# shivangchopra11/MedMoE

Measured on AMD Instinct MI355X. Metric: image-text pairs/sec at global batch 1024, higher is better.
Workload: dtype bf16; 1 GPU; cfg2: ViT-B/16 + 12-layer text tower (frozen), 8 experts top-2, 224x224x3 + 77 tokens, fwd+bwd+clip+Adam; global_batch=1024, per_gpu_batch=1024, parallelism=dp1

## Files before the change

include/medmoe_hip.h:

```cpp
#ifndef MEDMOE_HIP_H
#define MEDMOE_HIP_H
#include <hip/hip_runtime_api.h>
#ifdef __cplusplus
extern "C" {
#endif

int medmoe_attn_fwd(const void* qkv, void* out, float* lse, const unsigned char* key_mask, int B, int N, int H, int head_dim, hipStream_t stream);

int medmoe_attn_bwd(const void* qkv, const void* out, const void* dout, const float* lse, const unsigned char* key_mask, void* dqkv, float* delta, int B, int N, int H, int head_dim, hipStream_t stream);

int medmoe_patchify(const void* img, void* out, int B, int C, int H, int W, int patch, int in_f32, hipStream_t stream);
int medmoe_patchify_ld(const void* img, void* out, int B, int C, int H, int W, int patch, int in_f32, int ld, hipStream_t stream);

int medmoe_init_tokens(void* x, const float* cls, const float* pos, int B, int Nt, int D, hipStream_t stream);

int medmoe_pos_cls_grad(const void* dx, float* dpos, float* dcls, int B, int Nt, int D, hipStream_t stream);

int medmoe_text_embed_ln(const int* ids, const int* type_ids, const float* word, const float* pos, const float* type, const float* gamma, const float* beta, void* out, int B, int T, int D, int vocab, float eps, hipStream_t stream);

int medmoe_text_aggregate(const void* h0, const void* h1, const void* h2, const void* h3, int n_layers, const int* seg, void* word_bf16, float* word_f32, float* sent, int B, int T, int D, hipStream_t stream);

int medmoe_gemm_nt(const void* A, int lda, const void* B, int ldb, void* C, int ldc, int M, int N, int K, const float* bias, const void* residual, int ldr, void* aux, int ldaux, const int* a_rowmap, const int* c_rowmap, const int* tiles, const int* tile_count, int max_tiles, long long strideB, long long strideBias, float alpha, int epi, int out_f32, int col_perm, hipStream_t stream);

int medmoe_gemm_nt_tiles256(const void* A, int lda, const void* B, int ldb, void* C, int ldc, int M, int N, int K, const float* bias, const void* residual, int ldr, void* aux, int ldaux, const int* a_rowmap, const int* c_rowmap, const int* tiles, const int* tile_count, int max_tiles, long long strideB, long long strideBias, float alpha, int epi, int out_f32, int col_perm, hipStream_t stream);

int medmoe_gemm_tn(const void* G, int ldg, const void* X, int ldx, float* dW, int ldw, float* db, int M, int Nn, int Kk, const int* x_rowmap, const int* g_rowmap, const int* row_off, int n_groups, long long strideW, long long strideDb, int nsplit, hipStream_t stream);
int medmoe_gemm_tn_staged(const void* G, int ldg, const void* X, int ldx, float* dW, int ldw, float* db, int M, int Nn, int Kk, float* scratch, long long scratch_floats, hipStream_t stream);

int medmoe_ce_strided(const float* X, float* dX, int rows, int cols, long long rs, long long cs, int label_off, float xscale, float w, int accumulate, float* loss_acc, hipStream_t stream);

int medmoe_soft_xent_strided(const float* X, float* dX, const float* soft, int rows, int cols, long long rs, long long cs, float xscale, float t1, float t2, float w, int accumulate, float* loss_acc, hipStream_t stream);

int medmoe_hardneg_strided(const float* X, float* dX, int rows, int cols, long long rs, long long cs, float margin, float w, int accumulate, float* loss_acc, hipStream_t stream);

int medmoe_rownorm(const float* x, float* n, int rows, int D, hipStream_t stream);

int medmoe_cos_scale(float* S, const float* na, const float* nb, int M, int N, float eps, hipStream_t stream);

int medmoe_cos_scale_bwd(float* dC, const float* C, const float* na, const float* nb, float* ca, float* cb, int M, int N, float eps, hipStream_t stream);

int medmoe_add_rowscaled(float* dst, const float* src, const float* coef, int rows, int D, hipStream_t stream);

int medmoe_words_prep(const void* words, float* wn, void* wT, int Bc, int T, int Tp, int D, hipStream_t stream);

int medmoe_unpad_cast(const float* src, void* dst, int B, int HW, int HWp, int D, hipStream_t stream);

int medmoe_local_pair(const void* ctx, const void* words, const void* gmp, const float* wnorm, const int* cap_lens, const float* gsim, float* sim, void* dS, void* A, void* U, float* att, const void* a1_pre, const float* lse_pre, int B, int Bc, int HW, int T, int D, float temp1, float temp2, float eps, int backward, hipStream_t stream);

int medmoe_local_scores(const void* ctx, const void* words, const int* cap_lens, void* a1, float* lse, int B, int Bc, int HW, int T, int D, hipStream_t stream);

int medmoe_local_pair2(void* a1_io, const float* lse_pre, const void* gmp, const float* wnorm, const int* cap_lens, const float* gsim, float* sim, void* dS, void* U, float* att, int B, int Bc, int HW, int T, float temp1, float temp2, float eps, hipStream_t stream);

int medmoe_scale_blocks(void* X0, void* X1, const float* g, int B, int Bc, int HWp, int Tp, hipStream_t stream);

int medmoe_words_prep_ragged(const void* words, float* wn, void* wT, int Bc, int T, int Tp, int D, const int* col_of_cap, const int* tp_of_cap, long long ldw, hipStream_t stream);
int medmoe_local_scores_ragged(const void* ctx, const void* words, const int* cap_lens, void* a1, float* lse, int B, int Bc, int HW, int T, int D, const int* cap_list, int n_cap, int ntt, long long col_base, long long ldp, hipStream_t stream);
int medmoe_local_pair2_ragged(void* a1_io, const float* lse_pre, const void* gmp, const float* wnorm, const int* cap_lens, const float* gsim, float* sim, void* dS, void* U, int B, int Bc, int HW, int T, float temp1, float temp2, float eps, const int* cap_list, int n_cap, int ntt, long long col_base, long long ldp, hipStream_t stream);
int medmoe_scale_blocks_ragged(void* X0, void* X1, const float* g, int B, int Bc, int HWp, const int* cap_of_chunk, long long ld, hipStream_t stream);

int medmoe_local_pair3(const void* lp, void* dS, void* A, void* U, const float* lse, const void* gm, const float* wnorm, const int* cap_lens, const float* gsim, float* sim, float* att, float* stats, long long stat_rows, int B, int Bc, int HW, int T, float temp1, float temp2, float eps, const int* cap_list, int n_cap, int ntt, long long row_base, long long ld, long long bstride, int pw, float* d2, hipStream_t stream);
int medmoe_local_pair3_wgrad(const void* lp, void* dS, void* A, void* U, const float* lse, const void* gm, const float* wnorm, const int* cap_lens, const float* gsim, float* sim, float* att, float* stats, long long stat_rows, int B, int Bc, int HW, int T, float temp1, float temp2, float eps, const int* cap_list, int n_cap, int ntt, long long row_base, long long ld, long long bstride, int pw, float* d2, float* dwn, hipStream_t stream);
int medmoe_local_scores_t(const void* ctx, const void* words, const int* cap_lens, void* lpT, float* lse, int B, int Bc, int HW, int T, int D, const int* cap_list, int n_cap, int ntt, long long row_base, long long ld, long long bstride, hipStream_t stream);
int medmoe_gemm_tn_cols(const void* G, int ldg, const void* X, int ldx, float* dW, int ldw, int M, int Nn, int Kk, int n_groups, long long gcol_stride, long long xcol_stride, long long strideW, int g_chunk_w, long long g_chunk_stride, hipStream_t stream);

int medmoe_gemm_tn_gram(const void* A, int lda, const float* w, long long w_gstride, int w_ld, float* dW, int ldw, int M, int Nn, int n_groups, long long col_stride, long long strideW, hipStream_t stream);
int medmoe_local_sim_fwd(const void* ctx, const void* words, const int* cap_lens, const void* gm, const float* wnorm, float* sim, int B, int Bc, int HW, int T, int D, float temp1, float temp2, float eps, const int* cap_list, int n_cap, int ntt, hipStream_t stream);
int medmoe_local_sim_chunks(int n);
int medmoe_local_pair3_chunks(int n);
int medmoe_local_pair3_supported(int HW, int T);

int medmoe_segment_map(const void* ids, int ids64, const unsigned char* is_cont, const unsigned char* starts_bracket, int* seg, int* cap, int B, int T, int vocab, int sep_id, hipStream_t stream);

int medmoe_text_aggregate_bwd(const float* d_word, const float* d_sent, const int* seg, void* dH, int B, int T, int D, hipStream_t stream);
int medmoe_text_embed_ln_bwd(const int* ids, const int* type_ids, const float* word, const float* pos, const float* type, const float* gamma, const void* dy, float* dx, float* dgamma, float* dbeta, float* g_word, int B, int T, int D, int vocab, float eps, hipStream_t stream);

int medmoe_text_pack(const unsigned char* mask, int* tok_row, int* src_of_row, int* seq_off, int* count, int B, int T, hipStream_t stream);
int medmoe_text_embed_ln_packed(const int* ids, const int* type_ids, const float* word, const float* pos, const float* type, const float* gamma, const float* beta, void* out, int B, int T, int D, int vocab, float eps, const int* src_of_row, const int* count, hipStream_t stream);
int medmoe_text_aggregate_packed(const void* h0, const void* h1, const void* h2, const void* h3, int n_layers, const int* seg, const int* tok_row, void* word_bf16, float* word_f32, float* sent, int B, int T, int D, hipStream_t stream);
int medmoe_layernorm_fwd_rows(const void* x, const float* gamma, const float* beta, void* y, float* mean, float* rstd, int rows, int D, float eps, int out_f32, const int* rows_dev, hipStream_t stream);
int medmoe_attn_fwd_varlen(const void* qkv, void* out, float* lse, const int* seq_off, int B, int Nmax, int H, int head_dim, hipStream_t stream);
int medmoe_gemm_nt_rows(const void* A, int lda, const void* B, int ldb, void* C, int ldc, int M, int N, int K, const float* bias, const void* residual, int ldr, void* aux, int ldaux, float alpha, int epi, int out_f32, const int* m_dev, hipStream_t stream);

int medmoe_win_attn_fwd(const void* qkv, const float* bias, void* out, float* lse, int B, int H, int W, int C, int heads, int shift, hipStream_t stream);
int medmoe_win_attn_bwd(const void* qkv, const float* bias, const void* dout, const float* lse, void* dqkv, float* dbias, int B, int H, int W, int C, int heads, int shift, hipStream_t stream);
int medmoe_drop_path(const void* branch, const void* res, const float* scale, void* out, int B, long long per_sample, hipStream_t stream);
int medmoe_patch_merge(const void* src, void* dst, int B, int H, int W, int C, int scatter, hipStream_t stream);

int medmoe_preprocess(const void* const* src_ptrs, const int* src_hw, void* dst, int B, int Ho, int Wo, float rescale, const float* mean3, const float* std3, hipStream_t stream);
int medmoe_preprocess_bicubic(const void* const* src_ptrs, const long long* meta, const int* coef, void* tmp, void* dst, void* u8_out, int B, int Ho, int Wo, long long total_src_rows, float rescale, const float* mean3, const float* std3, hipStream_t stream);

int medmoe_local_geometry(int HW, int T, int* HWp, int* Tp, int* GW);
int medmoe_local_fast_path(int HW, int T);

int medmoe_local_gen_fwd_a(const void* lp, const int* cap_lens, void* A, int B, int Bc, int HW, int HWp, int T, int Tp, float temp1, long long ldp, hipStream_t stream);
int medmoe_local_gen_cos(const float* wc, const void* words, const float* wnorm, const int* cap_lens, float* sim, float* stats, float* sume, int B, int Bc, int T, int Tp, int D, float temp2, float eps, long long Kp, hipStream_t stream);
int medmoe_local_gen_dwctx(const float* wc, const void* words, const float* wnorm, const int* cap_lens, const float* gsim, const float* stats, const float* sume, void* dwc, int B, int Bc, int T, int Tp, int D, float temp2, float eps, long long Kp, hipStream_t stream);
int medmoe_local_gen_dwords(const float* wc, const void* words, const float* wnorm, const int* cap_lens, const float* gsim, const float* stats, const float* sume, const float* dws, float* d_words, int B, int Bc, int T, int Tp, int D, float temp2, float eps, long long Kp, hipStream_t stream);
int medmoe_local_gen_bwd_s(const void* lp, const void* A, void* dA_io, const int* cap_lens, int B, int Bc, int HW, int HWp, int T, int Tp, float temp1, long long ldp, hipStream_t stream);
int medmoe_unpad_cast2(const float* src, const float* src2, void* dst, int B, int HW, int HWp, int D, hipStream_t stream);

int medmoe_mean_tokens(const void* x, float* out, int B, int Nt, int D, int t0, int cnt, hipStream_t stream);

int medmoe_broadcast_tokens(const float* g, void* dy, int B, int Nt, int D, int t0, int cnt, float scale, hipStream_t stream);

int medmoe_router_fwd(const float* x, const float* w1, const float* b1, const float* w2, const float* b2, float* h, float* probs, int* idx, float* gates, int B, int Dv, int Hd, int E, int k, hipStream_t stream);

int medmoe_router_bwd(const float* probs, const float* h, const float* w2, const int* idx, const float* dgates, const int* labels, const float* dprobs_ext, float ce_scale, float* dlogits, float* dh, float* loss_acc, int B, int Hd, int E, int k, hipStream_t stream);

int medmoe_router_eval(const float* probs, const int* labels, float* loss_acc, int B, int E, hipStream_t stream);

int medmoe_sgemm(const float* A, const float* Bm, float* C, int M, int N, int K, long long sam, long long sak, long long sbk, long long sbn, long long ldc, float alpha, float beta, hipStream_t stream);

int medmoe_dispatch(const int* idx, int B, int k, int E, int P, int Nt, int* slot_of, int* item_of_slot, int* expert_of_slot, int* row_off, int* tiles, int* tile_count, int max_tiles, int* rowmap, hipStream_t stream);

int medmoe_scale_attn_fwd(const void* G, const void* H1, const float* w2, const float* b2, const int* expert_of_slot, int P, void* out, float* wts, int R, int Do, int Dh, hipStream_t stream);

int medmoe_combine_fwd(const void* expert_out, const int* slot_of, const float* gates, void* img_l, int B, int k, int P, int Do, hipStream_t stream);

int medmoe_scale_attn_bwd(const void* d_img_l, const float* d_img_g, const void* G, const void* H1, const float* wts, const float* w2, const void* expert_out, const int* expert_of_slot, const int* item_of_slot, const float* gates, int k, int P, void* dG, void* dH1, float* dw2, float* db2, float* dgate, int R, int Do, int Dh, hipStream_t stream);

int medmoe_lerp_tokens_fwd(const void* x, void* y, int n, int Pin, int Pout, int D, hipStream_t stream);
int medmoe_lerp_tokens_bwd(const void* dy, const void* relu_aux, void* dx, int n, int Pin, int Pout, int D, hipStream_t stream);
int medmoe_lerp_tokens_bwd2(const void* dy, const void* dy2, const void* relu_aux, void* dx, int n, int Pin, int Pout, int D, hipStream_t stream);

int medmoe_stage_grad_add(const void* dF, const int* slot_of, void* dx, int B, int k, int P, int Nt, int D, hipStream_t stream);

int medmoe_layernorm_fwd(const void* x, const float* gamma, const float* beta, void* y, float* mean, float* rstd, int rows, int D, float eps, int out_f32, hipStream_t stream);

int medmoe_layernorm_bwd(const void* dy, const void* x, const float* mean, const float* rstd, const float* gamma, const void* add, void* dx, float* dgamma, float* dbeta, int rows, int D, hipStream_t stream);

int medmoe_sumsq(const float* g, long long n, float* out, hipStream_t stream);
int medmoe_sumsq_det(const float* g, long long n, float* out, float* scratch, hipStream_t stream);

int medmoe_stream_fork(hipStream_t from, hipStream_t to);

int medmoe_adam_step(float* p, const float* g, float* m, float* v, void* p_bf16, long long n, double lr, double beta1, double beta2, double eps, double weight_decay, int step, const float* grad_normsq, float max_norm, float grad_scale, hipStream_t stream);

int medmoe_adam_groups_step(float* p, const float* g, float* m, float* v, void* p_bf16, long long n, const long long* run_end, const float* run_lr_mult, const float* run_wd_mult, int n_runs, double lr, double beta1, double beta2, double eps, double weight_decay, int decoupled, int step, const float* grad_normsq, float max_norm, float grad_scale, hipStream_t stream);

int medmoe_grad_pack_bf16(const float* g, void* out_bf16, long long n, float scale, hipStream_t stream);
int medmoe_sumsq_det_bf16(const void* g_bf16, long long n, float* out, float* scratch, hipStream_t stream);
int medmoe_adam_step_g16(float* p, const void* g_bf16, float* m, float* v, void* p_bf16, long long n, double lr, double beta1, double beta2, double eps, double weight_decay, int step, const float* grad_normsq, float max_norm, float grad_scale, hipStream_t stream);
int medmoe_adam_groups_step_g16(float* p, const void* g_bf16, float* m, float* v, void* p_bf16, long long n, const long long* run_end, const float* run_lr_mult, const float* run_wd_mult, int n_runs, double lr, double beta1, double beta2, double eps, double weight_decay, int decoupled, int step, const float* grad_normsq, float max_norm, float grad_scale, hipStream_t stream);

int medmoe_adam_step_ema(float* p, const float* g, float* m, float* v, void* p_bf16, long long n, double lr, double beta1, double beta2, double eps, double weight_decay, int step, const float* grad_normsq, float max_norm, float grad_scale, float* ema, float one_minus_decay, hipStream_t stream);
int medmoe_adam_groups_step_ema(float* p, const float* g, float* m, float* v, void* p_bf16, long long n, const long long* run_end, const float* run_lr_mult, const float* run_wd_mult, int n_runs, double lr, double beta1, double beta2, double eps, double weight_decay, int decoupled, int step, const float* grad_normsq, float max_norm, float grad_scale, float* ema, float one_minus_decay, hipStream_t stream);
int medmoe_adam_step_ema_g16(float* p, const void* g_bf16, float* m, float* v, void* p_bf16, long long n, double lr, double beta1, double beta2, double eps, double weight_decay, int step, const float* grad_normsq, float max_norm, float grad_scale, float* ema, float one_minus_decay, hipStream_t stream);
int medmoe_adam_groups_step_ema_g16(float* p, const void* g_bf16, float* m, float* v, void* p_bf16, long long n, const long long* run_end, const float* run_lr_mult, const float* run_wd_mult, int n_runs, double lr, double beta1, double beta2, double eps, double weight_decay, int decoupled, int step, const float* grad_normsq, float max_norm, float grad_scale, float* ema, float one_minus_decay, hipStream_t stream);

int medmoe_cast_bf16(const float* src, void* dst, long long n, hipStream_t stream);

int medmoe_transpose_many(const void* src, void* dst, const long long* table, int n_entries, int max_tiles, hipStream_t stream);

int medmoe_set_option(int key, int value);
int medmoe_last_gemm_nt_kernel(void);

int medmoe_quant_rows_e4m3(const void* x, int ldx, const int* rowmap, const float* colscale, const int* slot_expert, int rows_per_slot, void* q, float* s, int M, int K, hipStream_t stream);
int medmoe_quant_weights_e4m3(const float* w, void* q, void* qT, float* s, int G, int N, int K, hipStream_t stream);
int medmoe_gemm_fp8_grouped(const void* Aq, const float* sa, const void* Bq, const float* sb, const float* bias, void* C, int ldc, const void* residual, const void* aux, const int* tiles, const int* tile_count, int max_tiles, int N, int K, long long strideB, long long strideSb, long long strideBias, int epi, hipStream_t stream);

int medmoe_quant_rows_mx(const void* x, int ldx, const int* rowmap, void* q, void* s, int M, int K, hipStream_t stream);
int medmoe_quant_weights_mx(const float* w, void* q, void* sq, void* qT, void* sT, int G, int N, int K, hipStream_t stream);
int medmoe_gemm_mx_grouped(const void* Aq, const void* sa, const void* Bq, const void* sb, const float* bias, void* C, int ldc, const void* residual, const void* aux, void* Cq, void* Csq, const int* tiles, const int* tile_count, int max_tiles, int N, int K, long long strideB, long long strideSb, long long strideBias, int epi, hipStream_t stream);

int medmoe_dropout_mask(unsigned char* out_u8, long long rows, int cols, int cols_padded, long long seed, long long step, long long site, long long thresh, hipStream_t stream);
int medmoe_dropout_apply(const void* x, void* y, long long rows, int cols, int is_f32, long long seed, long long step, long long site, long long thresh, float scale, hipStream_t stream);
int medmoe_dropout_add_layernorm_fwd(const void* z, const void* residual, const float* gamma, const float* beta, void* x1, void* y, float* mean, float* rstd, int rows, int D, float eps, long long seed, long long step, long long site, long long thresh, float scale, hipStream_t stream);
int medmoe_attn_drop_fwd(const void* qkv, void* out, float* lse, const unsigned char* key_mask, int B, int N, int H, int head_dim, long long seed, long long step, long long site, long long thresh, float scale, hipStream_t stream);
int medmoe_attn_drop_bwd(const void* qkv, const void* out, const void* dout, const float* lse, const unsigned char* key_mask, void* dqkv, float* delta, int B, int N, int H, int head_dim, long long seed, long long step, long long site, long long thresh, float scale, hipStream_t stream);

int medmoe_drop_path_scales(float* out, const double* p_host, int n_sites, int B, long long sample0, long long seed, long long step, long long site0, hipStream_t stream);
int medmoe_scale_add_layernorm_fwd(const void* z, const void* residual, const float* scale, int rows_per_sample, const float* gamma, const float* beta, void* x1, void* y, float* mean, float* rstd, int rows, int D, float eps, hipStream_t stream);

int medmoe_gemm_tn_det(const void* G, int ldg, const void* X, int ldx, float* dW, int ldw, float* db, int M, int Nn, int Kk, const int* x_rowmap, const int* g_rowmap, const int* row_off, int n_groups, long long strideW, long long strideDb, float* scratch, long long scratch_floats, hipStream_t stream);
long long medmoe_gemm_tn_det_scratch(int M, int Nn, int Kk, int x_mapped, int g_mapped, int grouped, int n_groups);
int medmoe_gemm_tn_cols_det(const void* G, int ldg, const void* X, int ldx, float* dW, int ldw, int M, int Nn, int Kk, int n_groups, long long gcol_stride, long long xcol_stride, long long strideW, int g_chunk_w, long long g_chunk_stride, float* scratch, long long scratch_floats, hipStream_t stream);
long long medmoe_gemm_tn_cols_det_scratch(int M, int Nn, int Kk, int n_groups);
int medmoe_gemm_tn_gram_det(const void* A, int lda, const float* w, long long w_gstride, int w_ld, float* dW, int ldw, int M, int Nn, int n_groups, long long col_stride, long long strideW, hipStream_t stream);
int medmoe_layernorm_bwd_det(const void* dy, const void* x, const float* mean, const float* rstd, const float* gamma, const void* add, void* dx, float* dgamma, float* dbeta, int rows, int D, float* scratch, long long scratch_floats, hipStream_t stream);
long long medmoe_layernorm_bwd_det_scratch(int D);
int medmoe_scale_attn_bwd_det(const void* d_img_l, const float* d_img_g, const void* G, const void* H1, const float* wts, const float* w2, const void* expert_out, const int* expert_of_slot, const int* item_of_slot, const float* gates, int k, int P, void* dG, void* dH1, float* dw2, float* db2, float* dgate, int R, int Do, int Dh, const int* row_off, int E, float* scratch, long long scratch_floats, hipStream_t stream);
long long medmoe_scale_attn_bwd_det_scratch(int R, int P, int Dh);
int medmoe_router_bwd_det(const float* probs, const float* h, const float* w2, const int* idx, const float* dgates, const int* labels, const float* dprobs_ext, float ce_scale, float* dlogits, float* dh, float* loss_acc, int B, int Hd, int E, int k, float* parts, hipStream_t stream);
int medmoe_ce_strided_det(const float* X, float* dX, int rows, int cols, long long rs, long long cs, int label_off, float xscale, float w, int accumulate, float* loss_acc, float* parts, hipStream_t stream);
int medmoe_soft_xent_strided_det(const float* X, float* dX, const float* soft, int rows, int cols, long long rs, long long cs, float xscale, float t1, float t2, float w, int accumulate, float* loss_acc, float* parts, hipStream_t stream);
int medmoe_hardneg_strided_det(const float* X, float* dX, int rows, int cols, long long rs, long long cs, float margin, float w, int accumulate, float* loss_acc, float* parts, hipStream_t stream);
int medmoe_cos_scale_bwd_det(float* dC, const float* C, const float* na, const float* nb, float* ca, float* cb, int M, int N, float eps, hipStream_t stream);
long long medmoe_nondet_launches(void);

int medmoe_lora_fwd(const void* X, const void* A, const void* Bw, void* U, void* qkv, int ldq, int M, int D, int n, int c0, int c1, int c2, float s, long long seed, long long step, long long site, long long thresh, float scale, hipStream_t stream);
int medmoe_lora_bwd_dx(const void* dqkv, int ldq, const void* Bt, const void* At, void* dU, void* dy, int M, int D, int n, int c0, int c1, int c2, float s, long long seed, long long step, long long site, long long thresh, float scale, hipStream_t stream);
int medmoe_lora_bwd_wgrad(const void* dqkv, int ldq, const void* X, const void* U, const void* dU, float* gA, float* gB, float* scratch, long long scratch_floats, int M, int D, int n, int c0, int c1, int c2, float s, long long seed, long long step, long long site, long long thresh, float scale, hipStream_t stream);
long long medmoe_lora_wgrad_scratch(int M, int D, int n);
int medmoe_lora_merge(void* W, int ldw, const void* A, const void* Bw, int D, int n, int c0, int c1, int c2, float s, hipStream_t stream);

int medmoe_attn_bwd_varlen(const void* qkv, const void* out, const void* dout, const float* lse, const int* seq_off, void* dqkv, float* delta, int B, int Nmax, int H, int head_dim, hipStream_t stream);
int medmoe_layernorm_bwd_rows(const void* dy, const void* x, const float* mean, const float* rstd, const float* gamma, const void* add, void* dx, float* dgamma, float* dbeta, int rows, int D, const int* rows_dev, hipStream_t stream);
int medmoe_text_aggregate_bwd_packed(const float* d_word, const float* d_sent, const int* seg, const int* src_of_row, const int* count, void* dH, int B, int T, int D, hipStream_t stream);
int medmoe_text_embed_ln_bwd_packed(const int* ids, const int* type_ids, const float* word, const float* pos, const float* type, const float* gamma, const void* dy, float* dx, float* dgamma, float* dbeta, float* g_word, int B, int T, int D, int vocab, float eps, const int* src_of_row, const int* count, hipStream_t stream);
int medmoe_lora_fwd_rows(const void* X, const void* A, const void* Bw, void* U, void* qkv, int ldq, int M, int D, int n, int c0, int c1, int c2, float s, long long seed, long long step, long long site, long long thresh, float scale, const int* rows_dev, hipStream_t stream);
int medmoe_lora_bwd_dx_rows(const void* dqkv, int ldq, const void* Bt, const void* At, void* dU, void* dy, int M, int D, int n, int c0, int c1, int c2, float s, long long seed, long long step, long long site, long long thresh, float scale, const int* rows_dev, hipStream_t stream);
int medmoe_lora_bwd_wgrad_rows(const void* dqkv, int ldq, const void* X, const void* U, const void* dU, float* gA, float* gB, float* scratch, long long scratch_floats, int M, int D, int n, int c0, int c1, int c2, float s, long long seed, long long step, long long site, long long thresh, float scale, const int* rows_dev, hipStream_t stream);

#ifdef __cplusplus
}
#endif
#endif
```

medmoe_amd/csrc/attention.hip:

```cpp
#include "common.h"

#define HD 64

__device__ __forceinline__ int tpos(int r) {
  const int o = r & 31;
  return (r & ~31) + (((o & 15) >> 2) << 3) + ((o >> 4) << 2) + (o & 3);
}

template <int CNT, int RT>
__device__ __forceinline__ void fill_rowmajor(char* lds, const bf16_t* src, long long row_stride, int n_valid, int tid) {
  constexpr int PER = (CNT + RT - 1) / RT;
  uint4 v[PER];
#pragma unroll
  for (int i = 0; i < PER; ++i) {
    const int idx = min(tid + i * RT, CNT - 1);
    const int row = idx >> 3, c = idx & 7;
    v[i] = *(const uint4*)(src + (long long)min(row, n_valid - 1) * row_stride + c * 8);
  }
#pragma unroll
  for (int i = 0; i < PER; ++i) {
    const int idx = tid + i * RT;
    const int row = idx >> 3, c = idx & 7;
    if (idx < CNT) *(uint4*)(lds + row * 128 + ((c ^ (row & 7)) << 4)) = v[i];
  }
}

__device__ __forceinline__ void fill_transposed(char* lds, const bf16_t* src, long long row_stride, int n_valid,
                                                int stride_bytes, int tid) {
  for (int i = tid; i < (64 * stride_bytes) / 16; i += 256) *(uint4*)(lds + i * 16) = make_uint4(0, 0, 0, 0);
  __syncthreads();
  for (int idx = tid; idx < n_valid * 8; idx += 256) {
    const int row = idx >> 3, c = idx & 7;
    const uint4 v = *(const uint4*)(src + (long long)row * row_stride + c * 8);
    const uint32_t w[4] = {v.x, v.y, v.z, v.w};
    const int pos = tpos(row);
#pragma unroll
    for (int e = 0; e < 4; ++e) {
      *(bf16_t*)(lds + (c * 8 + 2 * e) * stride_bytes + pos * 2) = (bf16_t)(w[e] & 0xffff);
      *(bf16_t*)(lds + (c * 8 + 2 * e + 1) * stride_bytes + pos * 2) = (bf16_t)(w[e] >> 16);
    }
  }
}

__device__ __forceinline__ bf16x8_t tr_frag(const char* img, int row0, int col0, int lane) {
  const int q = (lane & 15) >> 2, pp = lane & 3;
  const int ra = row0 + 4 * (lane >> 4) + q, rb = ra + 16;
  const int col = col0 + 4 * pp;
  const int ch = col >> 3, within = (col & 7) << 1;
  const bf16x4_t lo = __builtin_amdgcn_ds_read_tr16_b64_v4bf16(
      (__attribute__((address_space(3))) bf16x4_t*)(img + ra * 128 + ((ch ^ (ra & 7)) << 4) + within));
  const bf16x4_t hi = __builtin_amdgcn_ds_read_tr16_b64_v4bf16(
      (__attribute__((address_space(3))) bf16x4_t*)(img + rb * 128 + ((ch ^ (rb & 7)) << 4) + within));
  return __builtin_shufflevector(lo, hi, 0, 1, 2, 3, 4, 5, 6, 7);
}

__device__ __forceinline__ bf16x8_t load_frag_global(const bf16_t* base, long long row_stride, int row, int chunk) {
  const uint4 v = *(const uint4*)(base + (long long)row * row_stride + chunk * 8);
  return __builtin_bit_cast(bf16x8_t, v);
}

__device__ __forceinline__ bf16x8_t pack_frag(const f32x4_t& a, const f32x4_t& b) {
  uint4 v;
  v.x = pack2bf(a[0], a[1]); v.y = pack2bf(a[2], a[3]);
  v.z = pack2bf(b[0], b[1]); v.w = pack2bf(b[2], b[3]);
  return __builtin_bit_cast(bf16x8_t, v);
}

template <int NKT>
struct AttnGeom {
  static constexpr int NKP = NKT * 16;
  static constexpr int KS = (NKT + 1) / 2;
  static constexpr int RMROWS = KS * 32;
  static constexpr int RM_BYTES = RMROWS * 128;
  static constexpr int FILL = RMROWS * 8;
};

#ifdef ATTN_TIMING
__device__ unsigned long long g_attn_timing[8];
#define ATTN_T(...) __VA_ARGS__
#else
#define ATTN_T(...)
#endif

template <int NKT, bool MASKED, int RT>
__global__ __launch_bounds__(RT, RT == 256 ? 2 : 4) void attn_fwd_kernel(const bf16_t* __restrict__ qkv, bf16_t* __restrict__ out,
                                                         float* __restrict__ lse, const unsigned char* __restrict__ key_mask,
                                                         int Nmax, int H, float scale, const int* __restrict__ seq_off) {
  using G = AttnGeom<NKT>;
  constexpr int CH = 8;
  constexpr int NCH = (NKT + CH - 1) / CH;
  __shared__ __attribute__((aligned(16))) char smem[2 * G::RM_BYTES + G::NKP * 4];
  char* sK = smem;
  char* sV = smem + G::RM_BYTES;
  float* sMask = (float*)(smem + 2 * G::RM_BYTES);
  const int tid = threadIdx.x, lane = tid & 63, wid = tid >> 6;
  const int b = blockIdx.x / H, h = blockIdx.x - b * H;
  const int D = H * HD;
  const long long rs = 3LL * D;
  const long long row0 = seq_off ? (long long)seq_off[b] : (long long)b * Nmax;
  const int N = seq_off ? max(1, min(seq_off[b + 1] - seq_off[b], Nmax)) : Nmax;
  const bf16_t* base = qkv + row0 * rs + h * HD;

  fill_rowmajor<G::FILL, RT>(sK, base + D, rs, N, tid);
  fill_rowmajor<G::FILL, RT>(sV, base + 2 * D, rs, N, tid);
  for (int k = tid; k < G::NKP; k += RT)
    sMask[k] = (k < N && (!key_mask || key_mask[(long long)b * Nmax + k])) ? 0.f : -INFINITY;
  __syncthreads();

  const int fr = lane & 15, g = lane >> 4;
  const int nqb = (N + 15) >> 4;
  const float c2 = scale * 1.44269504088896f;
  bf16x8_t qf[2], qn[2];
  {
    const int qc0 = min(wid * 16 + fr, N - 1);
    qf[0] = load_frag_global(base, rs, qc0, g);
    qf[1] = load_frag_global(base, rs, qc0, 4 + g);
  }
  for (int qb = wid; qb < nqb; qb += RT / 64) {
    const int q = qb * 16 + fr;
    {
      const int qcn = min((qb + RT / 64) * 16 + fr, N - 1);
      qn[0] = load_frag_global(base, rs, qcn, g);
      qn[1] = load_frag_global(base, rs, qcn, 4 + g);
    }
    float m = -INFINITY, lp = 0.f;
    f32x4_t o[4];
#pragma unroll
    for (int nd = 0; nd < 4; ++nd) o[nd] = (f32x4_t){0.f, 0.f, 0.f, 0.f};
#pragma unroll 1
    for (int c = 0; c < NCH; ++c) {
      const int kt0 = c * CH;
      f32x4_t s[CH];
#pragma unroll
      for (int u = 0; u < CH; ++u) {
        s[u] = (f32x4_t){0.f, 0.f, 0.f, 0.f};
        if (kt0 + u < NKT) {
          const char* kr = sK + ((kt0 + u) * 16 + fr) * 128;
#pragma unroll
          for (int ks = 0; ks < 2; ++ks) {
            const bf16x8_t kf = *(const bf16x8_t*)(kr + (((ks * 4 + g) ^ (fr & 7)) << 4));
            s[u] = __builtin_amdgcn_mfma_f32_16x16x32_bf16(kf, qf[ks], s[u], 0, 0, 0);
          }
        }
      }
      float alpha;
      f32x2_t l2 = {0.f, 0.f};
      if constexpr (MASKED) {
        float bm = -INFINITY;
#pragma unroll
        for (int u = 0; u < CH; ++u)
          if (kt0 + u < NKT) {
            const float4 mk = *(const float4*)(sMask + (kt0 + u) * 16 + g * 4);
            const f32x2_t t0 = (f32x2_t){s[u][0], s[u][1]} * c2 + (f32x2_t){mk.x, mk.y};
            const f32x2_t t1 = (f32x2_t){s[u][2], s[u][3]} * c2 + (f32x2_t){mk.z, mk.w};
            s[u][0] = t0[0]; s[u][1] = t0[1]; s[u][2] = t1[0]; s[u][3] = t1[1];
            bm = fmaxf(fmaxf(bm, fmaxf(t0[0], t0[1])), fmaxf(t1[0], t1[1]));
          }
        bm = fmaxf(bm, __shfl_xor(bm, 16, 64));
        bm = fmaxf(bm, __shfl_xor(bm, 32, 64));
        const float mn = fmaxf(m, bm);
        const float ms = (mn == -INFINITY) ? 0.f : mn;
        alpha = __builtin_amdgcn_exp2f(m - ms);
        m = mn;
#pragma unroll
        for (int u = 0; u < CH; ++u)
          if (kt0 + u < NKT) {
            const f32x2_t d0 = (f32x2_t){s[u][0], s[u][1]} - ms, d1 = (f32x2_t){s[u][2], s[u][3]} - ms;
            const f32x2_t e0 = {__builtin_amdgcn_exp2f(d0[0]), __builtin_amdgcn_exp2f(d0[1])};
            const f32x2_t e1 = {__builtin_amdgcn_exp2f(d1[0]), __builtin_amdgcn_exp2f(d1[1])};
            s[u][0] = e0[0]; s[u][1] = e0[1]; s[u][2] = e1[0]; s[u][3] = e1[1];
            l2 += e0 + e1;
          }
      } else {
        float bm = fmaxf(fmaxf(s[0][0], s[0][1]), fmaxf(s[0][2], s[0][3]));
#pragma unroll
        for (int u = 1; u < CH; ++u)
          if (kt0 + u < NKT) bm = fmaxf(fmaxf(bm, fmaxf(s[u][0], s[u][1])), fmaxf(s[u][2], s[u][3]));
        bm = fmaxf(bm, __shfl_xor(bm, 16, 64));
        bm = fmaxf(bm, __shfl_xor(bm, 32, 64));
        const float mn = fmaxf(m, bm * c2);
        alpha = __builtin_amdgcn_exp2f(m - mn);
        m = mn;
        const float nm = -mn;
#pragma unroll
        for (int u = 0; u < CH; ++u)
          if (kt0 + u < NKT) {
            const f32x2_t d0 = (f32x2_t){s[u][0], s[u][1]} * c2 + nm, d1 = (f32x2_t){s[u][2], s[u][3]} * c2 + nm;
            f32x2_t e0 = {__builtin_amdgcn_exp2f(d0[0]), __builtin_amdgcn_exp2f(d0[1])};
            f32x2_t e1 = {__builtin_amdgcn_exp2f(d1[0]), __builtin_amdgcn_exp2f(d1[1])};
            if ((kt0 + u) * 16 + 16 > N) {
              const int k0 = (kt0 + u) * 16 + g * 4;
              e0[0] = k0 < N ? e0[0] : 0.f; e0[1] = k0 + 1 < N ? e0[1] : 0.f;
              e1[0] = k0 + 2 < N ? e1[0] : 0.f; e1[1] = k0 + 3 < N ? e1[1] : 0.f;
            }
            s[u][0] = e0[0]; s[u][1] = e0[1]; s[u][2] = e1[0]; s[u][3] = e1[1];
            l2 += e0 + e1;
          }
      }
      lp = lp * alpha + l2[0] + l2[1];
#pragma unroll
      for (int nd = 0; nd < 4; ++nd) {
        if (c > 0) o[nd] *= alpha;
#pragma unroll
        for (int t = 0; t < CH / 2; ++t)
          if (kt0 + 2 * t < NKT) {
            const bf16x8_t pf = pack_frag(s[2 * t], s[2 * t + 1]);
            const bf16x8_t vf = tr_frag(sV, (kt0 + 2 * t) * 16, nd * 16, lane);
            o[nd] = __builtin_amdgcn_mfma_f32_16x16x32_bf16(vf, pf, o[nd], 0, 0, 0);
          }
      }
    }
    float l = lp;
    l += __shfl_xor(l, 16, 64);
    l += __shfl_xor(l, 32, 64);
    const float inv = l > 0.f ? 1.f / l : 0.f;
    if (q < N) {
      if (g == 0) lse[((long long)b * H + h) * Nmax + q] = (m + __log2f(l)) * 0.693147180559945f;
#pragma unroll
      for (int nd = 0; nd < 4; ++nd) {
        const f32x4_t v = o[nd] * inv;
        uint2 pk; pk.x = pack2bf(v[0], v[1]); pk.y = pack2bf(v[2], v[3]);
        *(uint2*)(out + (row0 + q) * D + h * HD + nd * 16 + g * 4) = pk;
      }
    }
    qf[0] = qn[0]; qf[1] = qn[1];
  }
}

template <int NKT, bool MASKED, int RT>
__global__ __launch_bounds__(RT, 4) void attn_bwd_dq_kernel(const bf16_t* __restrict__ qkv, const bf16_t* __restrict__ o,
                                                          const bf16_t* __restrict__ dout, const float* __restrict__ lse,
                                                          const unsigned char* __restrict__ key_mask,
                                                          bf16_t* __restrict__ dqkv, float* __restrict__ delta,
                                                          int Nmax, int H, float scale, const int* __restrict__ seq_off) {
  using G = AttnGeom<NKT>;
  __shared__ __attribute__((aligned(16))) char smem[2 * G::RM_BYTES + G::NKP * 4];
  char* sK = smem;
  char* sV = smem + G::RM_BYTES;
  float* sMask = (float*)(smem + 2 * G::RM_BYTES);
  const int tid = threadIdx.x, lane = tid & 63, wid = tid >> 6;
  const int b = blockIdx.x / H, h = blockIdx.x - b * H;
  const int D = H * HD;
  const long long rs = 3LL * D;
  const long long row0 = seq_off ? (long long)seq_off[b] : (long long)b * Nmax;
  const int N = seq_off ? max(1, min(seq_off[b + 1] - seq_off[b], Nmax)) : Nmax;
  const bf16_t* base = qkv + row0 * rs + h * HD;
  const bf16_t* obase = o + row0 * D + h * HD;
  const bf16_t* dobase = dout + row0 * D + h * HD;

  fill_rowmajor<G::FILL, RT>(sK, base + D, rs, N, tid);
  fill_rowmajor<G::FILL, RT>(sV, base + 2 * D, rs, N, tid);
  for (int k = tid; k < G::NKP; k += RT)
    sMask[k] = (k < N && (!key_mask || key_mask[(long long)b * Nmax + k])) ? 0.f : -INFINITY;
  __syncthreads();

  const int fr = lane & 15, g = lane >> 4;
  const int nqb = (N + 15) >> 4;
  bf16x8_t qf[2], dof[2], of[2], qn[2], don[2], on[2];
  {
    const int qc0 = min(wid * 16 + fr, N - 1);
#pragma unroll
    for (int ks = 0; ks < 2; ++ks) {
      qf[ks] = load_frag_global(base, rs, qc0, ks * 4 + g);
      dof[ks] = load_frag_global(dobase, D, qc0, ks * 4 + g);
      of[ks] = load_frag_global(obase, D, qc0, ks * 4 + g);
    }
  }
  for (int qb = wid; qb < nqb; qb += RT / 64) {
    const int q = qb * 16 + fr;
    const int qc = min(q, N - 1);
    {
      const int qcn = min((qb + RT / 64) * 16 + fr, N - 1);
#pragma unroll
      for (int ks = 0; ks < 2; ++ks) {
        qn[ks] = load_frag_global(base, rs, qcn, ks * 4 + g);
        don[ks] = load_frag_global(dobase, D, qcn, ks * 4 + g);
        on[ks] = load_frag_global(obase, D, qcn, ks * 4 + g);
      }
    }
    float dl = 0.f;
#pragma unroll
    for (int ks = 0; ks < 2; ++ks)
#pragma unroll
      for (int e = 0; e < 8; ++e) dl += (float)dof[ks][e] * (float)of[ks][e];
    dl += __shfl_xor(dl, 16, 64);
    dl += __shfl_xor(dl, 32, 64);
    const float c2 = scale * 1.44269504088896f;
    const float nL2 = -lse[((long long)b * H + h) * Nmax + qc] * 1.44269504088896f;
    if (g == 0 && q < N) delta[((long long)b * H + h) * Nmax + q] = dl;

    f32x4_t acc[4];
#pragma unroll
    for (int nd = 0; nd < 4; ++nd) acc[nd] = (f32x4_t){0.f, 0.f, 0.f, 0.f};
#pragma unroll 1
    for (int t = 0; t < G::KS; ++t) {
      f32x4_t ds[2];
#pragma unroll
      for (int u = 0; u < 2; ++u) {
        const int kt = 2 * t + u;
        ds[u] = (f32x4_t){0.f, 0.f, 0.f, 0.f};
        if (kt < NKT) {
          f32x4_t s = {0.f, 0.f, 0.f, 0.f}, dp = {0.f, 0.f, 0.f, 0.f};
          const char* kr = sK + (kt * 16 + fr) * 128;
          const char* vr = sV + (kt * 16 + fr) * 128;
#pragma unroll
          for (int ks = 0; ks < 2; ++ks) {
            const int off = ((ks * 4 + g) ^ (fr & 7)) << 4;
            s = __builtin_amdgcn_mfma_f32_16x16x32_bf16(*(const bf16x8_t*)(kr + off), qf[ks], s, 0, 0, 0);
            dp = __builtin_amdgcn_mfma_f32_16x16x32_bf16(*(const bf16x8_t*)(vr + off), dof[ks], dp, 0, 0, 0);
          }
          if (MASKED || kt * 16 + 16 > N) {
            const float4 mk = *(const float4*)(sMask + kt * 16 + g * 4);
            const float mkv[4] = {mk.x, mk.y, mk.z, mk.w};
#pragma unroll
            for (int r = 0; r < 4; ++r) ds[u][r] = __builtin_amdgcn_exp2f(s[r] * c2 + (mkv[r] + nL2)) * (dp[r] - dl);
          } else {
            const f32x2_t t0 = (f32x2_t){s[0], s[1]} * c2 + nL2, t1 = (f32x2_t){s[2], s[3]} * c2 + nL2;
            const f32x2_t g0 = (f32x2_t){dp[0], dp[1]} - dl, g1 = (f32x2_t){dp[2], dp[3]} - dl;
            const f32x2_t d0 = (f32x2_t){__builtin_amdgcn_exp2f(t0[0]), __builtin_amdgcn_exp2f(t0[1])} * g0;
            const f32x2_t d1 = (f32x2_t){__builtin_amdgcn_exp2f(t1[0]), __builtin_amdgcn_exp2f(t1[1])} * g1;
            ds[u] = (f32x4_t){d0[0], d0[1], d1[0], d1[1]};
          }
        }
      }
      const bf16x8_t dsf = pack_frag(ds[0], ds[1]);
#pragma unroll
      for (int nd = 0; nd < 4; ++nd) {
        const bf16x8_t ktf = tr_frag(sK, t * 32, nd * 16, lane);
        acc[nd] = __builtin_amdgcn_mfma_f32_16x16x32_bf16(ktf, dsf, acc[nd], 0, 0, 0);
      }
    }
    if (q < N) {
#pragma unroll
      for (int nd = 0; nd < 4; ++nd) {
        const f32x4_t v = acc[nd] * scale;
        uint2 pk; pk.x = pack2bf(v[0], v[1]); pk.y = pack2bf(v[2], v[3]);
        *(uint2*)(dqkv + (row0 + q) * rs + h * HD + nd * 16 + g * 4) = pk;
      }
    }
#pragma unroll
    for (int ks = 0; ks < 2; ++ks) { qf[ks] = qn[ks]; dof[ks] = don[ks]; of[ks] = on[ks]; }
  }
}

template <int NKT, int RT>
__global__ __launch_bounds__(RT, 4) void attn_bwd_dkv_kernel(const bf16_t* __restrict__ qkv, const bf16_t* __restrict__ dout,
                                                           const float* __restrict__ lse, const float* __restrict__ delta,
                                                           const unsigned char* __restrict__ key_mask,
                                                           bf16_t* __restrict__ dqkv, int Nmax, int H, float scale,
                                                           const int* __restrict__ seq_off) {
  using G = AttnGeom<NKT>;
  __shared__ __attribute__((aligned(16))) char smem[2 * G::RM_BYTES + G::NKP * 12];
  char* sQ = smem;
  char* sDO = smem + G::RM_BYTES;
  float* sMask = (float*)(smem + 2 * G::RM_BYTES);
  float* sLse = sMask + G::NKP;
  float* sDelta = sLse + G::NKP;
  const int tid = threadIdx.x, lane = tid & 63, wid = tid >> 6;
  const int b = blockIdx.x / H, h = blockIdx.x - b * H;
  const int D = H * HD;
  const long long rs = 3LL * D;
  const long long row0 = seq_off ? (long long)seq_off[b] : (long long)b * Nmax;
  const int N = seq_off ? max(1, min(seq_off[b + 1] - seq_off[b], Nmax)) : Nmax;
  const bf16_t* base = qkv + row0 * rs + h * HD;
  const bf16_t* dobase = dout + row0 * D + h * HD;

  fill_rowmajor<G::FILL, RT>(sQ, base, rs, N, tid);
  fill_rowmajor<G::FILL, RT>(sDO, dobase, D, N, tid);
  for (int k = tid; k < G::NKP; k += RT) {
    const bool valid = k < N;
    sMask[k] = (valid && (!key_mask || key_mask[(long long)b * Nmax + k])) ? 0.f : -INFINITY;
    sLse[k] = valid ? lse[((long long)b * H + h) * Nmax + k] * 1.44269504088896f : INFINITY;
    sDelta[k] = valid ? delta[((long long)b * H + h) * Nmax + k] : 0.f;
  }
  __syncthreads();

  const int fr = lane & 15, g = lane >> 4;
  const int nkb = (N + 15) >> 4;
  bf16x8_t kf[2], vf[2], kn[2], vn[2];
  {
    const int kc0 = min(wid * 16 + fr, N - 1);
#pragma unroll
    for (int ks = 0; ks < 2; ++ks) {
      kf[ks] = load_frag_global(base + D, rs, kc0, ks * 4 + g);
      vf[ks] = load_frag_global(base + 2 * D, rs, kc0, ks * 4 + g);
    }
  }
  for (int kb = wid; kb < nkb; kb += RT / 64) {
    const int key = kb * 16 + fr;
    {
      const int kcn = min((kb + RT / 64) * 16 + fr, N - 1);
#pragma unroll
      for (int ks = 0; ks < 2; ++ks) {
        kn[ks] = load_frag_global(base + D, rs, kcn, ks * 4 + g);
        vn[ks] = load_frag_global(base + 2 * D, rs, kcn, ks * 4 + g);
      }
    }
    const float mk = sMask[kb * 16 + fr];
    const float c2 = scale * 1.44269504088896f;
    f32x4_t dk[4], dv[4];
#pragma unroll
    for (int nd = 0; nd < 4; ++nd) { dk[nd] = (f32x4_t){0.f, 0.f, 0.f, 0.f}; dv[nd] = (f32x4_t){0.f, 0.f, 0.f, 0.f}; }

#pragma unroll 1
    for (int t = 0; t < G::KS; ++t) {
      f32x4_t pp[2], dss[2];
#pragma unroll
      for (int u = 0; u < 2; ++u) {
        const int qt = 2 * t + u;
        if (qt < NKT) {
          f32x4_t s = {0.f, 0.f, 0.f, 0.f}, dp = {0.f, 0.f, 0.f, 0.f};
          const char* qr = sQ + (qt * 16 + fr) * 128;
          const char* dr = sDO + (qt * 16 + fr) * 128;
#pragma unroll
          for (int ks = 0; ks < 2; ++ks) {
            const int off = ((ks * 4 + g) ^ (fr & 7)) << 4;
            s = __builtin_amdgcn_mfma_f32_16x16x32_bf16(*(const bf16x8_t*)(qr + off), kf[ks], s, 0, 0, 0);
            dp = __builtin_amdgcn_mfma_f32_16x16x32_bf16(*(const bf16x8_t*)(dr + off), vf[ks], dp, 0, 0, 0);
          }
          const float4 L4 = *(const float4*)(sLse + qt * 16 + g * 4);
          const float4 D4 = *(const float4*)(sDelta + qt * 16 + g * 4);
          const float Lv[4] = {L4.x, L4.y, L4.z, L4.w}, Dv[4] = {D4.x, D4.y, D4.z, D4.w};
          const f32x2_t t0 = (f32x2_t){s[0], s[1]} * c2 + (mk - (f32x2_t){Lv[0], Lv[1]});
          const f32x2_t t1 = (f32x2_t){s[2], s[3]} * c2 + (mk - (f32x2_t){Lv[2], Lv[3]});
          const f32x2_t p0 = {__builtin_amdgcn_exp2f(t0[0]), __builtin_amdgcn_exp2f(t0[1])};
          const f32x2_t p1 = {__builtin_amdgcn_exp2f(t1[0]), __builtin_amdgcn_exp2f(t1[1])};
          const f32x2_t d0 = p0 * ((f32x2_t){dp[0], dp[1]} - (f32x2_t){Dv[0], Dv[1]});
          const f32x2_t d1 = p1 * ((f32x2_t){dp[2], dp[3]} - (f32x2_t){Dv[2], Dv[3]});
          pp[u] = (f32x4_t){p0[0], p0[1], p1[0], p1[1]};
          dss[u] = (f32x4_t){d0[0], d0[1], d1[0], d1[1]};
        } else {
          pp[u] = (f32x4_t){0.f, 0.f, 0.f, 0.f};
          dss[u] = (f32x4_t){0.f, 0.f, 0.f, 0.f};
        }
      }
      const bf16x8_t pf = pack_frag(pp[0], pp[1]);
      const bf16x8_t dsf = pack_frag(dss[0], dss[1]);
#pragma unroll
      for (int nd = 0; nd < 4; ++nd) {
        const bf16x8_t dot = tr_frag(sDO, t * 32, nd * 16, lane);
        const bf16x8_t qt_ = tr_frag(sQ, t * 32, nd * 16, lane);
        dv[nd] = __builtin_amdgcn_mfma_f32_16x16x32_bf16(dot, pf, dv[nd], 0, 0, 0);
        dk[nd] = __builtin_amdgcn_mfma_f32_16x16x32_bf16(qt_, dsf, dk[nd], 0, 0, 0);
      }
    }
    if (key < N) {
      bf16_t* row = dqkv + (row0 + key) * rs + h * HD;
#pragma unroll
      for (int nd = 0; nd < 4; ++nd) {
        const f32x4_t kv = dk[nd] * scale;
        uint2 pk; pk.x = pack2bf(kv[0], kv[1]); pk.y = pack2bf(kv[2], kv[3]);
        *(uint2*)(row + D + nd * 16 + g * 4) = pk;
        pk.x = pack2bf(dv[nd][0], dv[nd][1]); pk.y = pack2bf(dv[nd][2], dv[nd][3]);
        *(uint2*)(row + 2 * D + nd * 16 + g * 4) = pk;
      }
    }
#pragma unroll
    for (int ks = 0; ks < 2; ++ks) { kf[ks] = kn[ks]; vf[ks] = vn[ks]; }
  }
}

#define SB 64
#define SB_BYTES (SB * 128)

__device__ __forceinline__ void stage_load(uint4 (&v)[2], const bf16_t* src, long long row_stride, int row0, int n_valid, int tid) {
#pragma unroll
  for (int i = 0; i < 2; ++i) {
    const int idx = tid + i * 256;
    const int row = idx >> 3, c = idx & 7;
    v[i] = *(const uint4*)(src + (long long)min(row0 + row, n_valid - 1) * row_stride + c * 8);
  }
}
__device__ __forceinline__ void stage_store(char* lds, const uint4 (&v)[2], int tid) {
#pragma unroll
  for (int i = 0; i < 2; ++i) {
    const int idx = tid + i * 256;
    const int row = idx >> 3, c = idx & 7;
    *(uint4*)(lds + row * 128 + ((c ^ (row & 7)) << 4)) = v[i];
  }
}
__device__ __forceinline__ bf16x8_t rm_frag(const char* img, int t16, int ks, int fr, int g) {
  return *(const bf16x8_t*)(img + (t16 * 16 + fr) * 128 + (((ks * 4 + g) ^ (fr & 7)) << 4));
}

template <bool MASKED>
__global__ __launch_bounds__(256) void attn_fwd_stream_kernel(const bf16_t* __restrict__ qkv, bf16_t* __restrict__ out,
                                                              float* __restrict__ lse, const unsigned char* __restrict__ key_mask,
                                                              int N, int H, int QB, float scale) {
  __shared__ __attribute__((aligned(16))) char smem[4 * SB_BYTES + 2 * SB * 4];
  const int tid = threadIdx.x, lane = tid & 63, wid = tid >> 6;
  const int fr = lane & 15, g = lane >> 4;
  const int id = xcd_remap(blockIdx.x, gridDim.x);
  const int bh = id / QB, qc = id - bh * QB;
  const int b = bh / H, h = bh - b * H;
  const int D = H * HD;
  const long long rs = 3LL * D;
  const bf16_t* base = qkv + (long long)b * N * rs + h * HD;
  const int q0 = qc * 64 + wid * 16;
  const bool active = q0 < N;
  const int q = q0 + fr;
  bf16x8_t qf[2];
  {
    const int qr = min(q, N - 1);
    qf[0] = load_frag_global(base, rs, qr, g);
    qf[1] = load_frag_global(base, rs, qr, 4 + g);
  }
  const int nkb = (N + SB - 1) / SB;
  auto bufK = [&](int i) { return smem + i * 2 * SB_BYTES; };
  auto bufV = [&](int i) { return smem + i * 2 * SB_BYTES + SB_BYTES; };
  float* sMaskAll = (float*)(smem + 4 * SB_BYTES);
  auto mask_of = [&](int key) -> float { return (key < N && (!key_mask || key_mask[(long long)b * N + key])) ? 0.f : -INFINITY; };
  uint4 kr[2], vr[2];
  stage_load(kr, base + D, rs, 0, N, tid);
  stage_load(vr, base + 2 * D, rs, 0, N, tid);
  stage_store(bufK(0), kr, tid); stage_store(bufV(0), vr, tid);
  if (tid < SB) sMaskAll[tid] = mask_of(tid);
  __syncthreads();

  const float c2 = scale * 1.44269504088896f;
  float m = -INFINITY, lp = 0.f;
  f32x4_t o[4];
#pragma unroll
  for (int nd = 0; nd < 4; ++nd) o[nd] = (f32x4_t){0.f, 0.f, 0.f, 0.f};
  for (int kb = 0; kb < nkb; ++kb) {
    const int cur = kb & 1;
    const bool more = kb + 1 < nkb;
    float mnext = 0.f;
    if (more) {
      stage_load(kr, base + D, rs, (kb + 1) * SB, N, tid);
      stage_load(vr, base + 2 * D, rs, (kb + 1) * SB, N, tid);
      if (tid < SB) mnext = mask_of((kb + 1) * SB + tid);
    }
    if (active) {
      const char* sK = bufK(cur);
      const char* sV = bufV(cur);
      const float* sM = sMaskAll + cur * SB;
      f32x4_t s[4];
#pragma unroll
      for (int kt = 0; kt < 4; ++kt) {
        s[kt] = (f32x4_t){0.f, 0.f, 0.f, 0.f};
#pragma unroll
        for (int ks = 0; ks < 2; ++ks) s[kt] = __builtin_amdgcn_mfma_f32_16x16x32_bf16(rm_frag(sK, kt, ks, fr, g), qf[ks], s[kt], 0, 0, 0);
      }
      float alpha;
      f32x2_t l2 = {0.f, 0.f};
      if constexpr (MASKED) {
        float bm = -INFINITY;
#pragma unroll
        for (int kt = 0; kt < 4; ++kt) {
          const float4 mk = *(const float4*)(sM + kt * 16 + g * 4);
          const f32x2_t t0 = (f32x2_t){s[kt][0], s[kt][1]} * c2 + (f32x2_t){mk.x, mk.y};
          const f32x2_t t1 = (f32x2_t){s[kt][2], s[kt][3]} * c2 + (f32x2_t){mk.z, mk.w};
          s[kt][0] = t0[0]; s[kt][1] = t0[1]; s[kt][2] = t1[0]; s[kt][3] = t1[1];
          bm = fmaxf(fmaxf(bm, fmaxf(t0[0], t0[1])), fmaxf(t1[0], t1[1]));
        }
        bm = fmaxf(bm, __shfl_xor(bm, 16, 64));
        bm = fmaxf(bm, __shfl_xor(bm, 32, 64));
        const float mn = fmaxf(m, bm);
        const float ms = (mn == -INFINITY) ? 0.f : mn;
        alpha = __builtin_amdgcn_exp2f(m - ms);
        m = mn;
#pragma unroll
        for (int kt = 0; kt < 4; ++kt) {
          const f32x2_t d0 = (f32x2_t){s[kt][0], s[kt][1]} - ms, d1 = (f32x2_t){s[kt][2], s[kt][3]} - ms;
          const f32x2_t e0 = {__builtin_amdgcn_exp2f(d0[0]), __builtin_amdgcn_exp2f(d0[1])};
          const f32x2_t e1 = {__builtin_amdgcn_exp2f(d1[0]), __builtin_amdgcn_exp2f(d1[1])};
          s[kt][0] = e0[0]; s[kt][1] = e0[1]; s[kt][2] = e1[0]; s[kt][3] = e1[1];
          l2 += e0 + e1;
        }
      } else {
        float bm = fmaxf(fmaxf(s[0][0], s[0][1]), fmaxf(s[0][2], s[0][3]));
#pragma unroll
        for (int kt = 1; kt < 4; ++kt) bm = fmaxf(fmaxf(bm, fmaxf(s[kt][0], s[kt][1])), fmaxf(s[kt][2], s[kt][3]));
        bm = fmaxf(bm, __shfl_xor(bm, 16, 64));
        bm = fmaxf(bm, __shfl_xor(bm, 32, 64));
        const float mn = fmaxf(m, bm * c2);
        alpha = __builtin_amdgcn_exp2f(m - mn);
        m = mn;
        const float nm = -mn;
        const bool tail = kb * SB + SB > N;
#pragma unroll
        for (int kt = 0; kt < 4; ++kt) {
          const f32x2_t d0 = (f32x2_t){s[kt][0], s[kt][1]} * c2 + nm, d1 = (f32x2_t){s[kt][2], s[kt][3]} * c2 + nm;
          f32x2_t e0 = {__builtin_amdgcn_exp2f(d0[0]), __builtin_amdgcn_exp2f(d0[1])};
          f32x2_t e1 = {__builtin_amdgcn_exp2f(d1[0]), __builtin_amdgcn_exp2f(d1[1])};
          if (tail) {
            const int k0 = kb * SB + kt * 16 + g * 4;
            e0[0] = k0 < N ? e0[0] : 0.f; e0[1] = k0 + 1 < N ? e0[1] : 0.f;
            e1[0] = k0 + 2 < N ? e1[0] : 0.f; e1[1] = k0 + 3 < N ? e1[1] : 0.f;
          }
          s[kt][0] = e0[0]; s[kt][1] = e0[1]; s[kt][2] = e1[0]; s[kt][3] = e1[1];
          l2 += e0 + e1;
        }
      }
      lp = lp * alpha + l2[0] + l2[1];
      bf16x8_t pf[2];
      pf[0] = pack_frag(s[0], s[1]);
      pf[1] = pack_frag(s[2], s[3]);
#pragma unroll
      for (int nd = 0; nd < 4; ++nd) {
        o[nd] *= alpha;
#pragma unroll
        for (int t = 0; t < 2; ++t) o[nd] = __builtin_amdgcn_mfma_f32_16x16x32_bf16(tr_frag(sV, t * 32, nd * 16, lane), pf[t], o[nd], 0, 0, 0);
      }
    }
    if (more) {
      stage_store(bufK(cur ^ 1), kr, tid); stage_store(bufV(cur ^ 1), vr, tid);
      if (tid < SB) sMaskAll[(cur ^ 1) * SB + tid] = mnext;
    }
    __syncthreads();
  }
  if (!active) return;
  float l = lp;
  l += __shfl_xor(l, 16, 64);
  l += __shfl_xor(l, 32, 64);
  const float inv = l > 0.f ? 1.f / l : 0.f;
  if (q < N) {
    if (g == 0) lse[((long long)b * H + h) * N + q] = (m + __log2f(l)) * 0.693147180559945f;
#pragma unroll
    for (int nd = 0; nd < 4; ++nd) {
      const f32x4_t v = o[nd] * inv;
      uint2 pk; pk.x = pack2bf(v[0], v[1]); pk.y = pack2bf(v[2], v[3]);
      *(uint2*)(out + ((long long)b * N + q) * D + h * HD + nd * 16 + g * 4) = pk;
    }
  }
}

template <bool MASKED>
__global__ __launch_bounds__(256) void attn_bwd_dq_stream_kernel(const bf16_t* __restrict__ qkv, const bf16_t* __restrict__ o,
                                                                 const bf16_t* __restrict__ dout, const float* __restrict__ lse,
                                                                 const unsigned char* __restrict__ key_mask,
                                                                 bf16_t* __restrict__ dqkv, float* __restrict__ delta,
                                                                 int N, int H, int QB, float scale) {
  __shared__ __attribute__((aligned(16))) char smem[4 * SB_BYTES + 2 * SB * 4];
  const int tid = threadIdx.x, lane = tid & 63, wid = tid >> 6;
  const int fr = lane & 15, g = lane >> 4;
  const int id = xcd_remap(blockIdx.x, gridDim.x);
  const int bh = id / QB, qc = id - bh * QB;
  const int b = bh / H, h = bh - b * H;
  const int D = H * HD;
  const long long rs = 3LL * D;
  const bf16_t* base = qkv + (long long)b * N * rs + h * HD;
  const bf16_t* obase = o + (long long)b * N * D + h * HD;
  const bf16_t* dobase = dout + (long long)b * N * D + h * HD;
  const int q0 = qc * 64 + wid * 16;
  const bool active = q0 < N;
  const int q = q0 + fr, qr = min(q, N - 1);
  bf16x8_t qf[2], dof[2];
  float dl = 0.f;
  {
    bf16x8_t of[2];
#pragma unroll
    for (int ks = 0; ks < 2; ++ks) {
      qf[ks] = load_frag_global(base, rs, qr, ks * 4 + g);
      dof[ks] = load_frag_global(dobase, D, qr, ks * 4 + g);
      of[ks] = load_frag_global(obase, D, qr, ks * 4 + g);
    }
#pragma unroll
    for (int ks = 0; ks < 2; ++ks)
#pragma unroll
      for (int e = 0; e < 8; ++e) dl += (float)dof[ks][e] * (float)of[ks][e];
    dl += __shfl_xor(dl, 16, 64);
    dl += __shfl_xor(dl, 32, 64);
  }
  const float c2 = scale * 1.44269504088896f;
  const float nL2 = -lse[((long long)b * H + h) * N + qr] * 1.44269504088896f;
  if (active && g == 0 && q < N) delta[((long long)b * H + h) * N + q] = dl;

  const int nkb = (N + SB - 1) / SB;
  auto bufK = [&](int i) { return smem + i * 2 * SB_BYTES; };
  auto bufV = [&](int i) { return smem + i * 2 * SB_BYTES + SB_BYTES; };
  float* sMaskAll = (float*)(smem + 4 * SB_BYTES);
  auto mask_of = [&](int key) -> float { return (key < N && (!key_mask || key_mask[(long long)b * N + key])) ? 0.f : -INFINITY; };
  uint4 kr[2], vr[2];
  stage_load(kr, base + D, rs, 0, N, tid);
  stage_load(vr, base + 2 * D, rs, 0, N, tid);
  stage_store(bufK(0), kr, tid); stage_store(bufV(0), vr, tid);
  if (tid < SB) sMaskAll[tid] = mask_of(tid);
  __syncthreads();
  f32x4_t acc[4];
#pragma unroll
  for (int nd = 0; nd < 4; ++nd) acc[nd] = (f32x4_t){0.f, 0.f, 0.f, 0.f};
  for (int kb = 0; kb < nkb; ++kb) {
    const int cur = kb & 1;
    const bool more = kb + 1 < nkb;
    float mnext = 0.f;
    if (more) {
      stage_load(kr, base + D, rs, (kb + 1) * SB, N, tid);
      stage_load(vr, base + 2 * D, rs, (kb + 1) * SB, N, tid);
      if (tid < SB) mnext = mask_of((kb + 1) * SB + tid);
    }
    if (active) {
      const char* sK = bufK(cur);
      const char* sV = bufV(cur);
      const float* sM = sMaskAll + cur * SB;
      f32x4_t ds[4];
#pragma unroll
      for (int kt = 0; kt < 4; ++kt) {
        f32x4_t s = {0.f, 0.f, 0.f, 0.f}, dp = {0.f, 0.f, 0.f, 0.f};
#pragma unroll
        for (int ks = 0; ks < 2; ++ks) {
          s = __builtin_amdgcn_mfma_f32_16x16x32_bf16(rm_frag(sK, kt, ks, fr, g), qf[ks], s, 0, 0, 0);
          dp = __builtin_amdgcn_mfma_f32_16x16x32_bf16(rm_frag(sV, kt, ks, fr, g), dof[ks], dp, 0, 0, 0);
        }
        if (MASKED || kb * SB + SB > N) {
          const float4 mk = *(const float4*)(sM + kt * 16 + g * 4);
          const float mkv[4] = {mk.x, mk.y, mk.z, mk.w};
#pragma unroll
          for (int r = 0; r < 4; ++r) ds[kt][r] = __builtin_amdgcn_exp2f(s[r] * c2 + (mkv[r] + nL2)) * (dp[r] - dl);
        } else {
          const f32x2_t t0 = (f32x2_t){s[0], s[1]} * c2 + nL2, t1 = (f32x2_t){s[2], s[3]} * c2 + nL2;
          const f32x2_t d0 = (f32x2_t){__builtin_amdgcn_exp2f(t0[0]), __builtin_amdgcn_exp2f(t0[1])} * ((f32x2_t){dp[0], dp[1]} - dl);
          const f32x2_t d1 = (f32x2_t){__builtin_amdgcn_exp2f(t1[0]), __builtin_amdgcn_exp2f(t1[1])} * ((f32x2_t){dp[2], dp[3]} - dl);
          ds[kt] = (f32x4_t){d0[0], d0[1], d1[0], d1[1]};
        }
      }
      const bf16x8_t dsf0 = pack_frag(ds[0], ds[1]), dsf1 = pack_frag(ds[2], ds[3]);
#pragma unroll
      for (int nd = 0; nd < 4; ++nd) {
        acc[nd] = __builtin_amdgcn_mfma_f32_16x16x32_bf16(tr_frag(sK, 0, nd * 16, lane), dsf0, acc[nd], 0, 0, 0);
        acc[nd] = __builtin_amdgcn_mfma_f32_16x16x32_bf16(tr_frag(sK, 32, nd * 16, lane), dsf1, acc[nd], 0, 0, 0);
      }
    }
    if (more) {
      stage_store(bufK(cur ^ 1), kr, tid); stage_store(bufV(cur ^ 1), vr, tid);
      if (tid < SB) sMaskAll[(cur ^ 1) * SB + tid] = mnext;
    }
    __syncthreads();
  }
  if (active && q < N) {
#pragma unroll
    for (int nd = 0; nd < 4; ++nd) {
      const f32x4_t v = acc[nd] * scale;
      uint2 pk; pk.x = pack2bf(v[0], v[1]); pk.y = pack2bf(v[2], v[3]);
      *(uint2*)(dqkv + ((long long)b * N + q) * rs + h * HD + nd * 16 + g * 4) = pk;
    }
  }
}

__global__ __launch_bounds__(256) void attn_bwd_dkv_stream_kernel(const bf16_t* __restrict__ qkv, const bf16_t* __restrict__ dout,
                                                                  const float* __restrict__ lse, const float* __restrict__ delta,
                                                                  const unsigned char* __restrict__ key_mask,
                                                                  bf16_t* __restrict__ dqkv, int N, int H, int QB, float scale) {
  __shared__ __attribute__((aligned(16))) char smem[4 * SB_BYTES + 4 * SB * 4];
  const int tid = threadIdx.x, lane = tid & 63, wid = tid >> 6;
  const int fr = lane & 15, g = lane >> 4;
  const int id = xcd_remap(blockIdx.x, gridDim.x);
  const int bh = id / QB, kc = id - bh * QB;
  const int b = bh / H, h = bh - b * H;
  const int D = H * HD;
  const long long rs = 3LL * D;
  const bf16_t* base = qkv + (long long)b * N * rs + h * HD;
  const bf16_t* dobase = dout + (long long)b * N * D + h * HD;
  const float* lrow = lse + ((long long)b * H + h) * N;
  const float* drow = delta + ((long long)b * H + h) * N;
  const int k0 = kc * 64 + wid * 16;
  const bool active = k0 < N;
  const int key = k0 + fr, kr_ = min(key, N - 1);
  bf16x8_t kf[2], vf[2];
#pragma unroll
  for (int ks = 0; ks < 2; ++ks) {
    kf[ks] = load_frag_global(base + D, rs, kr_, ks * 4 + g);
    vf[ks] = load_frag_global(base + 2 * D, rs, kr_, ks * 4 + g);
  }
  const float mk = (key < N && (!key_mask || key_mask[(long long)b * N + key])) ? 0.f : -INFINITY;
  const float c2 = scale * 1.44269504088896f;
  const int nqb = (N + SB - 1) / SB;
  auto bufQ = [&](int i) { return smem + i * 2 * SB_BYTES; };
  auto bufD = [&](int i) { return smem + i * 2 * SB_BYTES + SB_BYTES; };
  float* sL = (float*)(smem + 4 * SB_BYTES);
  float* sDl = sL + 2 * SB;
  uint4 qr[2], dr[2];
  stage_load(qr, base, rs, 0, N, tid);
  stage_load(dr, dobase, D, 0, N, tid);
  stage_store(bufQ(0), qr, tid); stage_store(bufD(0), dr, tid);
  if (tid < SB) { sL[tid] = tid < N ? lrow[tid] * 1.44269504088896f : INFINITY; sDl[tid] = tid < N ? drow[tid] : 0.f; }
  __syncthreads();
  f32x4_t dk[4], dv[4];
#pragma unroll
  for (int nd = 0; nd < 4; ++nd) { dk[nd] = (f32x4_t){0.f, 0.f, 0.f, 0.f}; dv[nd] = (f32x4_t){0.f, 0.f, 0.f, 0.f}; }
  for (int qb = 0; qb < nqb; ++qb) {
    const int cur = qb & 1;
    const bool more = qb + 1 < nqb;
    float ln = 0.f, dn = 0.f;
    if (more) {
      stage_load(qr, base, rs, (qb + 1) * SB, N, tid);
      stage_load(dr, dobase, D, (qb + 1) * SB, N, tid);
      if (tid < SB) {
        const int qq = (qb + 1) * SB + tid;
        ln = qq < N ? lrow[qq] * 1.44269504088896f : INFINITY; dn = qq < N ? drow[qq] : 0.f;
      }
    }
    if (active) {
      const char* sQ = bufQ(cur);
      const char* sDO = bufD(cur);
      const float* cL = sL + cur * SB;
      const float* cD = sDl + cur * SB;
      f32x4_t pp[4], dss[4];
#pragma unroll
      for (int qt = 0; qt < 4; ++qt) {
        f32x4_t s = {0.f, 0.f, 0.f, 0.f}, dp = {0.f, 0.f, 0.f, 0.f};
#pragma unroll
        for (int ks = 0; ks < 2; ++ks) {
          s = __builtin_amdgcn_mfma_f32_16x16x32_bf16(rm_frag(sQ, qt, ks, fr, g), kf[ks], s, 0, 0, 0);
          dp = __builtin_amdgcn_mfma_f32_16x16x32_bf16(rm_frag(sDO, qt, ks, fr, g), vf[ks], dp, 0, 0, 0);
        }
        const float4 L4 = *(const float4*)(cL + qt * 16 + g * 4);
        const float4 D4 = *(const float4*)(cD + qt * 16 + g * 4);
        const float Lv[4] = {L4.x, L4.y, L4.z, L4.w}, Dv[4] = {D4.x, D4.y, D4.z, D4.w};
        const f32x2_t t0 = (f32x2_t){s[0], s[1]} * c2 + (mk - (f32x2_t){Lv[0], Lv[1]});
        const f32x2_t t1 = (f32x2_t){s[2], s[3]} * c2 + (mk - (f32x2_t){Lv[2], Lv[3]});
        const f32x2_t p0 = {__builtin_amdgcn_exp2f(t0[0]), __builtin_amdgcn_exp2f(t0[1])};
        const f32x2_t p1 = {__builtin_amdgcn_exp2f(t1[0]), __builtin_amdgcn_exp2f(t1[1])};
        const f32x2_t d0 = p0 * ((f32x2_t){dp[0], dp[1]} - (f32x2_t){Dv[0], Dv[1]});
        const f32x2_t d1 = p1 * ((f32x2_t){dp[2], dp[3]} - (f32x2_t){Dv[2], Dv[3]});
        pp[qt] = (f32x4_t){p0[0], p0[1], p1[0], p1[1]};
        dss[qt] = (f32x4_t){d0[0], d0[1], d1[0], d1[1]};
      }
#pragma unroll
      for (int t = 0; t < 2; ++t) {
        const bf16x8_t pf = pack_frag(pp[2 * t], pp[2 * t + 1]);
        const bf16x8_t dsf = pack_frag(dss[2 * t], dss[2 * t + 1]);
#pragma unroll
        for (int nd = 0; nd < 4; ++nd) {
          dv[nd] = __builtin_amdgcn_mfma_f32_16x16x32_bf16(tr_frag(sDO, t * 32, nd * 16, lane), pf, dv[nd], 0, 0, 0);
          dk[nd] = __builtin_amdgcn_mfma_f32_16x16x32_bf16(tr_frag(sQ, t * 32, nd * 16, lane), dsf, dk[nd], 0, 0, 0);
        }
      }
    }
    if (more) {
      stage_store(bufQ(cur ^ 1), qr, tid); stage_store(bufD(cur ^ 1), dr, tid);
      if (tid < SB) { sL[(cur ^ 1) * SB + tid] = ln; sDl[(cur ^ 1) * SB + tid] = dn; }
    }
    __syncthreads();
  }
  if (active && key < N) {
    bf16_t* row = dqkv + ((long long)b * N + key) * rs + h * HD;
#pragma unroll
    for (int nd = 0; nd < 4; ++nd) {
      const f32x4_t kv = dk[nd] * scale;
      uint2 pk; pk.x = pack2bf(kv[0], kv[1]); pk.y = pack2bf(kv[2], kv[3]);
      *(uint2*)(row + D + nd * 16 + g * 4) = pk;
      pk.x = pack2bf(dv[nd][0], dv[nd][1]); pk.y = pack2bf(dv[nd][2], dv[nd][3]);
      *(uint2*)(row + 2 * D + nd * 16 + g * 4) = pk;
    }
  }
}

int g_attn_resident = 1;
int g_attn_rt13 = 0;

static int pick_nkt(int N) {
  if (N <= 80) return 5;
  if (N <= 208) return 13;
  if (N <= 272) return 17;
  if (N <= 592) return 37;
  return 0;
}

template <int K, int RT>
static void launch_fwd(const void* qkv, void* out, float* lse, const unsigned char* key_mask, int B, int N, int H, float scale, hipStream_t stream) {
  if (key_mask) hipLaunchKernelGGL((attn_fwd_kernel<K, true, RT>), dim3(B * H), dim3(RT), 0, stream, (const bf16_t*)qkv, (bf16_t*)out, lse, key_mask, N, H, scale, (const int*)nullptr);
  else hipLaunchKernelGGL((attn_fwd_kernel<K, false, RT>), dim3(B * H), dim3(RT), 0, stream, (const bf16_t*)qkv, (bf16_t*)out, lse, key_mask, N, H, scale, (const int*)nullptr);
}
template <int K, int RT>
static void launch_bwd(const void* qkv, const void* out, const void* dout, const float* lse, const unsigned char* key_mask, void* dqkv,
                       float* delta, int B, int N, int H, float scale, hipStream_t stream) {
  if (key_mask) hipLaunchKernelGGL((attn_bwd_dq_kernel<K, true, RT>), dim3(B * H), dim3(RT), 0, stream, (const bf16_t*)qkv, (const bf16_t*)out,
                                   (const bf16_t*)dout, lse, key_mask, (bf16_t*)dqkv, delta, N, H, scale, (const int*)nullptr);
  else hipLaunchKernelGGL((attn_bwd_dq_kernel<K, false, RT>), dim3(B * H), dim3(RT), 0, stream, (const bf16_t*)qkv, (const bf16_t*)out,
                          (const bf16_t*)dout, lse, key_mask, (bf16_t*)dqkv, delta, N, H, scale, (const int*)nullptr);
  hipLaunchKernelGGL((attn_bwd_dkv_kernel<K, RT>), dim3(B * H), dim3(RT), 0, stream, (const bf16_t*)qkv, (const bf16_t*)dout, lse, delta,
                     key_mask, (bf16_t*)dqkv, N, H, scale, (const int*)nullptr);
}

extern "C" int medmoe_attn_fwd(const void* qkv, void* out, float* lse, const unsigned char* key_mask,
                               int B, int N, int H, int head_dim, hipStream_t stream) {
  if (!qkv || !out || !lse) return MM_ERR_ARG;
  if (head_dim != HD || B <= 0 || H <= 0 || N <= 0) return MM_ERR_SHAPE;
  const int nkt = pick_nkt(N);
  const float scale = 0.125f;
  if (!g_attn_resident || !nkt) {
    const int QB = (N + SB - 1) / SB;
    if (key_mask) hipLaunchKernelGGL(attn_fwd_stream_kernel<true>, dim3(B * H * QB), dim3(256), 0, stream, (const bf16_t*)qkv, (bf16_t*)out,
                                     lse, key_mask, N, H, QB, scale);
    else hipLaunchKernelGGL(attn_fwd_stream_kernel<false>, dim3(B * H * QB), dim3(256), 0, stream, (const bf16_t*)qkv, (bf16_t*)out,
                            lse, key_mask, N, H, QB, scale);
    return mm_check_launch();
  }
  if (nkt == 5) launch_fwd<5, 256>(qkv, out, lse, key_mask, B, N, H, scale, stream);
  else if (nkt == 13 && (g_attn_rt13 == 448 || (g_attn_rt13 == 0 && B * H >= 4096))) launch_fwd<13, 448>(qkv, out, lse, key_mask, B, N, H, scale, stream);
  else if (nkt == 13) launch_fwd<13, 512>(qkv, out, lse, key_mask, B, N, H, scale, stream);
  else if (nkt == 17) launch_fwd<17, 512>(qkv, out, lse, key_mask, B, N, H, scale, stream);
  else launch_fwd<37, 1024>(qkv, out, lse, key_mask, B, N, H, scale, stream);
  return mm_check_launch();
}

extern "C" int medmoe_attn_fwd_varlen(const void* qkv, void* out, float* lse, const int* seq_off, int B, int Nmax, int H, int head_dim,
                                      hipStream_t stream) {
  if (!qkv || !out || !lse || !seq_off) return MM_ERR_ARG;
  if (head_dim != HD || B <= 0 || H <= 0 || Nmax <= 0 || Nmax > 80) return MM_ERR_SHAPE;
  hipLaunchKernelGGL((attn_fwd_kernel<5, false, 256>), dim3(B * H), dim3(256), 0, stream, (const bf16_t*)qkv, (bf16_t*)out, lse,
                     (const unsigned char*)nullptr, Nmax, H, 0.125f, seq_off);
  return mm_check_launch();
}

extern "C" int medmoe_attn_bwd(const void* qkv, const void* out, const void* dout, const float* lse,
                               const unsigned char* key_mask, void* dqkv, float* delta, int B, int N,
                               int H, int head_dim, hipStream_t stream) {
  if (!qkv || !out || !dout || !lse || !dqkv || !delta) return MM_ERR_ARG;
  if (head_dim != HD || B <= 0 || H <= 0 || N <= 0) return MM_ERR_SHAPE;
  const int nkt = pick_nkt(N);
  const float scale = 0.125f;
  if (!g_attn_resident || !nkt) {
    const int QB = (N + SB - 1) / SB;
    if (key_mask) hipLaunchKernelGGL(attn_bwd_dq_stream_kernel<true>, dim3(B * H * QB), dim3(256), 0, stream, (const bf16_t*)qkv,
                                     (const bf16_t*)out, (const bf16_t*)dout, lse, key_mask, (bf16_t*)dqkv, delta, N, H, QB, scale);
    else hipLaunchKernelGGL(attn_bwd_dq_stream_kernel<false>, dim3(B * H * QB), dim3(256), 0, stream, (const bf16_t*)qkv,
                            (const bf16_t*)out, (const bf16_t*)dout, lse, key_mask, (bf16_t*)dqkv, delta, N, H, QB, scale);
    hipLaunchKernelGGL(attn_bwd_dkv_stream_kernel, dim3(B * H * QB), dim3(256), 0, stream, (const bf16_t*)qkv, (const bf16_t*)dout,
                       lse, delta, key_mask, (bf16_t*)dqkv, N, H, QB, scale);
    return mm_check_launch();
  }
  if (nkt == 5) launch_bwd<5, 256>(qkv, out, dout, lse, key_mask, dqkv, delta, B, N, H, scale, stream);
  else if (nkt == 13 && g_attn_rt13 == 448) launch_bwd<13, 448>(qkv, out, dout, lse, key_mask, dqkv, delta, B, N, H, scale, stream);
  else if (nkt == 13) launch_bwd<13, 512>(qkv, out, dout, lse, key_mask, dqkv, delta, B, N, H, scale, stream);
  else if (nkt == 17) launch_bwd<17, 512>(qkv, out, dout, lse, key_mask, dqkv, delta, B, N, H, scale, stream);
  else launch_bwd<37, 1024>(qkv, out, dout, lse, key_mask, dqkv, delta, B, N, H, scale, stream);
  return mm_check_launch();
}

extern "C" int medmoe_attn_bwd_varlen(const void* qkv, const void* out, const void* dout, const float* lse, const int* seq_off, void* dqkv,
                                      float* delta, int B, int Nmax, int H, int head_dim, hipStream_t stream) {
  if (!qkv || !out || !dout || !lse || !seq_off || !dqkv || !delta) return MM_ERR_ARG;
  if (head_dim != HD || B <= 0 || H <= 0 || Nmax <= 0 || Nmax > 80) return MM_ERR_SHAPE;
  hipLaunchKernelGGL((attn_bwd_dq_kernel<5, false, 256>), dim3(B * H), dim3(256), 0, stream, (const bf16_t*)qkv, (const bf16_t*)out,
                     (const bf16_t*)dout, lse, (const unsigned char*)nullptr, (bf16_t*)dqkv, delta, Nmax, H, 0.125f, seq_off);
  hipLaunchKernelGGL((attn_bwd_dkv_kernel<5, 256>), dim3(B * H), dim3(256), 0, stream, (const bf16_t*)qkv, (const bf16_t*)dout, lse, delta,
                     (const unsigned char*)nullptr, (bf16_t*)dqkv, Nmax, H, 0.125f, seq_off);
  return mm_check_launch();
}
```

medmoe_amd/csrc/gemm.hip:

```cpp
#include "common.h"
#include "det_plan.h"
#include <utility>

#define BM 128
#define BN 128
#define BK 64

__device__ __attribute__((aligned(256))) bf16_t g_zero_page[2048];

struct GemmNTArgs {
  const bf16_t* A; const bf16_t* B; void* C;
  const float* bias; const bf16_t* residual; bf16_t* aux;
  const int* a_rowmap; const int* c_rowmap; const int4* tiles; const int* tile_count;
  long long strideB; long long strideBias;
  int M, N, K, lda, ldb, ldc, ldr, ldaux;
  int n_tiles_n, max_tiles_m;
  float alpha; int epi; int out_f32; int col_perm;
  const int* m_dev;
};

static int g_use_nt256 = 1, g_use_nt512 = 1, g_use_tn512 = 1, g_tn_rows = 1024, g_nt_max_grid = 256, g_use_scores512 = 1, g_use_nt4w = 1, g_use_tn4w = 1, g_tn_min_rows = 2048, g_tn_rows4w = 0, g_scores_skip_epi = 0;
#ifdef NT_EXPERIMENT
__device__ int g_nt_dbg_skip = 0;
#define NT_X(...) __VA_ARGS__
#else
#define NT_X(...)
#endif
#ifdef NT_TIMING
__device__ unsigned long long g_nt_timing[8 * 8];
#define NT_T(...) __VA_ARGS__
__device__ __forceinline__ long long nt_clk() {
  __builtin_amdgcn_sched_barrier(0); const long long c = clock64(); __builtin_amdgcn_sched_barrier(0); return c;
}
#else
#define NT_T(...)
#endif
extern int g_attn_resident;
extern int g_sa_rows;
extern int g_attn_rt13;
static int g_last_nt_kernel = -1;
extern "C" int medmoe_last_gemm_nt_kernel() { return g_last_nt_kernel; }
extern int g_ln_one_row;
int g_use_nt_direct = 1;
extern "C" int medmoe_set_option(int key, int value) {
  if (key == 16) { g_ln_one_row = value; return MM_OK; }
  if (key == 17) { g_use_nt_direct = value; return MM_OK; }
  if (key == 1) { g_use_nt256 = value; return MM_OK; }
  if (key == 2) { g_use_nt512 = value; return MM_OK; }
  if (key == 3) { g_use_tn512 = value; return MM_OK; }
  if (key == 4 && value >= 256) { g_tn_rows = value; return MM_OK; }
  if (key == 5 && value >= 1 && value <= 256) { g_nt_max_grid = value; return MM_OK; }
  if (key == 6) { g_use_scores512 = value; return MM_OK; }
  if (key == 7) { g_use_nt4w = value; return MM_OK; }
  if (key == 8) { g_use_tn4w = value; return MM_OK; }
  if (key == 9 && value >= 64) { g_tn_min_rows = value; return MM_OK; }
  if (key == 12) { g_scores_skip_epi = value; return MM_OK; }
  if (key == 15 && (value == 0 || value == 448 || value == 512)) { g_attn_rt13 = value; return MM_OK; }
  if (key == 13 && value >= 0) { g_sa_rows = value; return MM_OK; }
  if (key == 11) { g_attn_resident = value; return MM_OK; }
  if (key == 10 && value >= 0) { g_tn_rows4w = value; return MM_OK; }
  return MM_ERR_ARG;
}

enum { EPI_NONE = 0, EPI_GELU = 1, EPI_RELU = 2, EPI_MUL_DGELU = 3, EPI_MUL_DRELU = 4, EPI_GELU_DAUX = 5, EPI_MUL_AUX = 6 };

struct ParkedTile {
  uint4 c[8];
  int m_base, n_base, n_items, next;
};

typedef unsigned u32x4e_t __attribute__((ext_vector_type(4)));
template <bool PARK, int TM0 = 0, int TMS = 4, int TN0 = 0, int TNS = 4, bool LDSX = false>
__device__ __forceinline__ int nt_epilogue(const GemmNTArgs& p, f32x4_t (&acc)[TMS][TNS], int m_base, int m_end,
                                           int n_base, int group, int frag_row, int frag_q, ParkedTile* park, unsigned lds_x = 0u) {
  int n_stores = 0;
  const int pg = ((frag_q & 1) << 1) | (frag_q >> 1);
  long long mc[4];
  bool mok[4];
#pragma unroll
  for (int tm = 0; tm < 4; ++tm) {
    const int m = m_base + tm * 16 + frag_row;
    mok[tm] = m < m_end;
    const int mr = min(m, m_end - 1);
    mc[tm] = p.c_rowmap ? (long long)p.c_rowmap[mr] : (long long)mr;
  }
  int nn[4];
  bool nok[4];
#pragma unroll
  for (int tn = 0; tn < 4; ++tn) {
    const int n = n_base + tn * 16 + pg * 4;
    nok[tn] = n < p.N;
    nn[tn] = min(n, p.N - 4);
  }
  float4 b4[4];
  if (p.bias) {
    const float* bias = p.bias + (long long)group * p.strideBias;
#pragma unroll
    for (int tn = 0; tn < 4; ++tn) b4[tn] = *(const float4*)(bias + nn[tn]);
  }
  uint2 res[4][4], axv[4][4];
  if (p.residual) {
#pragma unroll
    for (int tm = 0; tm < 4; ++tm)
#pragma unroll
      for (int tn = 0; tn < 4; ++tn) res[tm][tn] = *(const uint2*)(p.residual + mc[tm] * p.ldr + nn[tn]);
  }
  const bool mul_epi = p.epi == EPI_MUL_DGELU || p.epi == EPI_MUL_DRELU || p.epi == EPI_MUL_AUX;
  if (mul_epi) {
#pragma unroll
    for (int tm = 0; tm < 4; ++tm)
#pragma unroll
      for (int tn = 0; tn < 4; ++tn) axv[tm][tn] = *(const uint2*)(p.aux + mc[tm] * p.ldaux + nn[tn]);
  }
  const bool wide = !p.out_f32 && !p.col_perm && (p.N & 7) == 0;
  const bool upper = frag_q >= 2;
  auto store_pair = [&](bf16_t* base, long long ld, int tm, int j, uint2 lo, uint2 hi, bool is_aux) {
    auto r0 = __builtin_amdgcn_permlane32_swap(lo.x, hi.x, false, false);
    auto r1 = __builtin_amdgcn_permlane32_swap(lo.y, hi.y, false, false);
    if constexpr (PARK) {
      if (!is_aux) { park->c[tm * 2 + j] = make_uint4(r0[0], r1[0], r0[1], r1[1]); return; }
    }
    if constexpr (LDSX) {
      const int row_l = (tm & 1) * 16 + frag_row, slot = (2 * j + (upper ? 1 : 0)) * 2 + (frag_q & 1);
      const unsigned a = lds_x + (is_aux ? 4096u : 0u) + row_l * 128 + ((slot ^ ((row_l >> 1) & 7)) << 4);
      const u32x4e_t d = {(unsigned)r0[0], (unsigned)r1[0], (unsigned)r0[1], (unsigned)r1[1]};
      asm volatile("ds_write_b128 %0, %1" :: "v"(a), "v"(d) : "memory");
      return;
    }
    const int col = n_base + (2 * j + (upper ? 1 : 0)) * 16 + (frag_q & 1) * 8;
    const bool pred = mok[tm] && col < p.N;
    n_stores += (__ballot(pred) != 0ull) ? 1 : 0;
    if (pred) *(uint4*)(base + mc[tm] * ld + col) = make_uint4(r0[0], r1[0], r0[1], r1[1]);
  };
#pragma unroll
  for (int tm = 0; tm < 4; ++tm) {
    uint2 o[4], zz[4];
#pragma unroll
    for (int tn = 0; tn < 4; ++tn) {
      float v[4];
#pragma unroll
      for (int r = 0; r < 4; ++r) v[r] = acc[TM0 + tm][TN0 + tn][r] * p.alpha;
      if (p.bias) { v[0] += b4[tn].x; v[1] += b4[tn].y; v[2] += b4[tn].z; v[3] += b4[tn].w; }
      const bool ok = mok[tm] && nok[tn];
      zz[tn] = make_uint2(0u, 0u);
      if (p.epi == EPI_GELU_DAUX) {
        f32x2_t g0, g1, d0, d1;
        gelu_and_grad2((f32x2_t){v[0], v[1]}, g0, d0); gelu_and_grad2((f32x2_t){v[2], v[3]}, g1, d1);
        v[0] = g0[0]; v[1] = g0[1]; v[2] = g1[0]; v[3] = g1[1];
        if (p.aux) {
          zz[tn].x = pack2bf(d0[0], d0[1]); zz[tn].y = pack2bf(d1[0], d1[1]);
          if (!wide) { n_stores += (__ballot(ok) != 0ull) ? 1 : 0; if (ok) *(uint2*)(p.aux + mc[tm] * p.ldaux + nn[tn]) = zz[tn]; }
        }
      } else       if (p.epi == EPI_GELU) {
        if (p.aux) {
          zz[tn].x = pack2bf(v[0], v[1]); zz[tn].y = pack2bf(v[2], v[3]);
          if (!wide) { n_stores += (__ballot(ok) != 0ull) ? 1 : 0; if (ok) *(uint2*)(p.aux + mc[tm] * p.ldaux + nn[tn]) = zz[tn]; }
        }
        {
          const f32x2_t g0 = gelu2((f32x2_t){v[0], v[1]}), g1 = gelu2((f32x2_t){v[2], v[3]});
          v[0] = g0[0]; v[1] = g0[1]; v[2] = g1[0]; v[3] = g1[1];
        }
      } else if (p.epi == EPI_RELU) {
#pragma unroll
        for (int r = 0; r < 4; ++r) v[r] = fmaxf(v[r], 0.f);
      }
      if (p.residual) {
        const uint2 z = res[tm][tn];
        v[0] += bf2f((bf16_t)(z.x & 0xffff)); v[1] += bf2f((bf16_t)(z.x >> 16));
        v[2] += bf2f((bf16_t)(z.y & 0xffff)); v[3] += bf2f((bf16_t)(z.y >> 16));
      }
      if (mul_epi) {
        const uint2 z = axv[tm][tn];
        const float zf[4] = {bf2f((bf16_t)(z.x & 0xffff)), bf2f((bf16_t)(z.x >> 16)),
                             bf2f((bf16_t)(z.y & 0xffff)), bf2f((bf16_t)(z.y >> 16))};
        if (p.epi == EPI_MUL_DGELU) {
          const f32x2_t d0 = dgelu2((f32x2_t){zf[0], zf[1]}), d1 = dgelu2((f32x2_t){zf[2], zf[3]});
          v[0] *= d0[0]; v[1] *= d0[1]; v[2] *= d1[0]; v[3] *= d1[1];
        } else if (p.epi == EPI_MUL_AUX) {
#pragma unroll
          for (int r = 0; r < 4; ++r) v[r] *= zf[r];
        } else {
#pragma unroll
          for (int r = 0; r < 4; ++r) v[r] *= zf[r] > 0.f ? 1.f : 0.f;
        }
      }
      o[tn].x = pack2bf(v[0], v[1]); o[tn].y = pack2bf(v[2], v[3]);
      if (!wide) n_stores += (__ballot(ok) != 0ull) ? 1 : 0;
      if (!wide && ok) {
        const int n = nn[tn];
        const int ns = p.col_perm ? ((n & ~31) + ((((n & 31) & 15) >> 2) << 3) + (((n & 31) >> 4) << 2)) : n;
        if (p.out_f32) *(float4*)((float*)p.C + mc[tm] * p.ldc + ns) = make_float4(v[0], v[1], v[2], v[3]);
        else *(uint2*)((bf16_t*)p.C + mc[tm] * p.ldc + ns) = o[tn];
      }
    }
    if (wide) {
#pragma unroll
      for (int j = 0; j < 2; ++j) {
        store_pair((bf16_t*)p.C, p.ldc, tm, j, o[2 * j], o[2 * j + 1], false);
        if ((p.epi == EPI_GELU || p.epi == EPI_GELU_DAUX) && p.aux) store_pair(p.aux, p.ldaux, tm, j, zz[2 * j], zz[2 * j + 1], true);
      }
      if constexpr (LDSX) {
        if (tm & 1) {
          const bool has_aux = (p.epi == EPI_GELU || p.epi == EPI_GELU_DAUX) && p.aux;
          const int lane = frag_q * 16 + frag_row, c8 = lane & 7;
          const int col = n_base + c8 * 8;
          u32x4e_t vc[4], va[4];
#pragma unroll
          for (int i = 0; i < 4; ++i) {
            const int row_l = i * 8 + (lane >> 3);
            const unsigned a = lds_x + row_l * 128 + ((c8 ^ ((row_l >> 1) & 7)) << 4);
            asm volatile("ds_read_b128 %0, %1" : "=v"(vc[i]) : "v"(a));
            if (has_aux) asm volatile("ds_read_b128 %0, %1 offset:4096" : "=v"(va[i]) : "v"(a));
          }
          asm volatile("s_waitcnt lgkmcnt(0)" ::: "memory");
#pragma unroll
          for (int i = 0; i < 4; ++i) {
            const int m = m_base + (tm - 1) * 16 + i * 8 + (lane >> 3);
            const bool pred = m < m_end && col < p.N;
            const int ns = (__ballot(pred) != 0ull) ? 1 : 0;
            n_stores += has_aux ? 2 * ns : ns;
            if (pred) {
              __builtin_nontemporal_store(vc[i], (u32x4e_t*)((bf16_t*)p.C + (long long)m * p.ldc + col));
              if (has_aux) __builtin_nontemporal_store(va[i], (u32x4e_t*)(p.aux + (long long)m * p.ldaux + col));
            }
          }
        }
      }
    }
  }
  if constexpr (PARK) { park->m_base = m_base; park->n_base = n_base; park->next = 0; park->n_items = 8; }
  return n_stores;
}

__device__ __forceinline__ int park_store_next(const GemmNTArgs& p, ParkedTile& pk, int m_end, int frag_row, int frag_q) {
  const int item = pk.next++;
  const uint4 v = pk.c[0];
#pragma unroll
  for (int i = 0; i < 7; ++i) pk.c[i] = pk.c[i + 1];
  const int tm = item >> 1, j = item & 1;
  const int row = pk.m_base + tm * 16 + frag_row;
  const int col = pk.n_base + (2 * j + (frag_q >= 2 ? 1 : 0)) * 16 + (frag_q & 1) * 8;
  const bool pred = row < m_end && col < p.N;
  if (__builtin_amdgcn_readfirstlane(__ballot(pred) != 0ull ? 1 : 0) == 0) return 0;
  if (pred) *(uint4*)((bf16_t*)p.C + (long long)row * p.ldc + col) = v;
  return 1;
}

__device__ __forceinline__ void wait_vmcnt(int n) {
  if (n == 6) asm volatile("s_waitcnt vmcnt(6)" ::: "memory");
  else if (n == 7) asm volatile("s_waitcnt vmcnt(7)" ::: "memory");
  else if (n == 8) asm volatile("s_waitcnt vmcnt(8)" ::: "memory");
  else if (n >= 16) asm volatile("s_waitcnt vmcnt(16)" ::: "memory");
  else if (n >= 14) asm volatile("s_waitcnt vmcnt(14)" ::: "memory");
  else if (n >= 8) asm volatile("s_waitcnt vmcnt(8)" ::: "memory");
  else asm volatile("s_waitcnt vmcnt(0)" ::: "memory");
}

__device__ __forceinline__ void wait_vmcnt_plus6(int n) {
  switch (n) {
#define WV(k, k6) case k: asm volatile("s_waitcnt vmcnt(" #k6 ")" ::: "memory"); break;
    WV(1, 7) WV(2, 8) WV(3, 9) WV(4, 10) WV(5, 11) WV(6, 12) WV(7, 13) WV(8, 14) WV(9, 15) WV(10, 16) WV(11, 17) WV(12, 18)
    WV(13, 19) WV(14, 20) WV(15, 21) WV(16, 22)
#undef WV
    default: asm volatile("s_waitcnt vmcnt(6)" ::: "memory"); break;
  }
}

__global__ __launch_bounds__(256, 2) void gemm_nt_kernel(GemmNTArgs p) {
  __shared__ __attribute__((aligned(16))) char smem[2 * 32768];
  const int tid = threadIdx.x, lane = tid & 63, wid = tid >> 6;
  const int wm = wid >> 1, wn = wid & 1;
  const int frag_row = lane & 15, frag_q = lane >> 4, swz = lane & 7;
  const int G = gridDim.x;
  const int my = xcd_remap(blockIdx.x, G);
  if (!p.tiles && p.m_dev) { p.M = min(*p.m_dev, p.M); p.max_tiles_m = (p.M + BM - 1) / BM; }
  const int n_tiles_m = p.tiles ? min(*p.tile_count, p.max_tiles_m) : p.max_tiles_m;
  const int total = n_tiles_m * p.n_tiles_n;
  const int nt = (p.K + BK - 1) / BK;
  const bool khalf = (p.K & 32) != 0;
  const int tail_adj = (khalf && (((lane & 7) ^ ((lane >> 3) & 7)) >= 4)) ? -32 : 0;

  struct Tile { int group, m0, m_end, n0; };
  auto decode = [&](int id) -> Tile {
    Tile t;
    const int tile_m = id / p.n_tiles_n, tile_n = id - tile_m * p.n_tiles_n;
    if (p.tiles) { const int4 q = p.tiles[tile_m]; t.group = q.x; t.m0 = q.y; t.m_end = q.z; }
    else { t.group = 0; t.m0 = tile_m * BM; t.m_end = p.M; }
    t.n0 = tile_n * BN;
    return t;
  };
  const bf16_t* asrc[4];
  const bf16_t* bsrc[4];
  auto setup = [&](const Tile& t) {
    const bf16_t* Bg = p.B + (long long)t.group * p.strideB;
#pragma unroll
    for (int i = 0; i < 4; ++i) {
      const int row = i * 32 + wid * 8 + (lane >> 3);
      const int c = (lane & 7) ^ (row & 7);
      int ra = min(t.m0 + row, t.m_end - 1);
      if (p.a_rowmap) ra = p.a_rowmap[ra];
      asrc[i] = p.A + (long long)ra * p.lda + c * 8;
      const int rb = min(t.n0 + row, p.N - 1);
      bsrc[i] = Bg + (long long)rb * p.ldb + c * 8;
    }
  };
  auto stage = [&](int buf, int ks) {
    char* sA = smem + buf * 32768 + wid * 1024;
    char* sB = sA + 16384;
    const int k0 = ks * BK + ((ks == nt - 1) ? tail_adj : 0);
#pragma unroll
    for (int i = 0; i < 4; ++i) {
      __builtin_amdgcn_global_load_lds(GLB_PTR(asrc[i] + k0), LDS_PTR(sA + i * 4096), 16, 0, 0);
      __builtin_amdgcn_global_load_lds(GLB_PTR(bsrc[i] + k0), LDS_PTR(sB + i * 4096), 16, 0, 0);
    }
  };

  f32x4_t acc[4][4];
  auto zero_acc = [&]() {
#pragma unroll
    for (int i = 0; i < 4; ++i)
#pragma unroll
      for (int j = 0; j < 4; ++j) acc[i][j] = (f32x4_t){0.f, 0.f, 0.f, 0.f};
  };
  const int sig = ((((frag_row >> 2) & 1) << 1 | (frag_row >> 3)) << 2) | (frag_row & 3);
  auto compute = [&](int buf, int nks) {
    const char* sA = smem + buf * 32768 + (wm * 64 + frag_row) * 128;
    const char* sB = smem + buf * 32768 + 16384 + (wn * 64 + sig) * 128;
#pragma unroll
    for (int ks = 0; ks < 2; ++ks) {
      if (ks >= nks) break;
      const int coff = ((ks * 4 + frag_q) ^ swz) * 16;
      const int coffb = ((ks * 4 + frag_q) ^ (sig & 7)) * 16;
      bf16x8_t af[4], bf[4];
#pragma unroll
      for (int t = 0; t < 4; ++t) {
        af[t] = *(const bf16x8_t*)(sA + t * 2048 + coff);
        bf[t] = *(const bf16x8_t*)(sB + t * 2048 + coffb);
      }
#pragma unroll
      for (int tm = 0; tm < 4; ++tm)
#pragma unroll
        for (int tn = 0; tn < 4; ++tn)
          acc[tm][tn] = __builtin_amdgcn_mfma_f32_16x16x32_bf16(bf[tn], af[tm], acc[tm][tn], 0, 0, 0);
    }
  };
  auto epilogue = [&](const Tile& t) -> int { return nt_epilogue<false>(p, acc, t.m0 + wm * 64, t.m_end, t.n0 + wn * 64, t.group, frag_row, frag_q, nullptr); };

  int id = my;
  if (id >= total) return;
  Tile cur_t = decode(id);
  setup(cur_t);
  zero_acc();
  stage(0, 0);
  asm volatile("s_waitcnt vmcnt(0)" ::: "memory");
  __syncthreads();
  int cur = 0;
  while (true) {
    const int nid = id + G;
    const bool has_next = nid < total;
    Tile next_t = cur_t;
// ... 2328 lines not shown
```

Measured before the change: 4807 pairs/s.

## Make attention kernels persistent with prefetched next-item K/V handover

Converts attention forward and backward kernels into persistent grids sized from occupancy times CU count. Each block loops over (batch, head) items and prefetches the next item's K/V (or Q/dO), mask, lse and delta rows into registers while finishing the current one, then hands them over to LDS. This targets block launch overhead and the exposed global-load latency at the start of each block for short sequences with many items. It also changes launch bounds for the 256-thread forward kernel to 4 waves/SIMD, which raises register pressure, and adds a grid-cap option plus a query for the last grid size.

```diff
diff --git a/include/medmoe_hip.h b/include/medmoe_hip.h
--- a/include/medmoe_hip.h
+++ b/include/medmoe_hip.h
@@ -154,6 +154,7 @@
 
 int medmoe_set_option(int key, int value);
 int medmoe_last_gemm_nt_kernel(void);
+int medmoe_attn_last_grid(int which);
 
 int medmoe_quant_rows_e4m3(const void* x, int ldx, const int* rowmap, const float* colscale, const int* slot_expert, int rows_per_slot, void* q, float* s, int M, int K, hipStream_t stream);
 int medmoe_quant_weights_e4m3(const float* w, void* q, void* qT, float* s, int G, int N, int K, hipStream_t stream);
diff --git a/medmoe_amd/csrc/attention.hip b/medmoe_amd/csrc/attention.hip
--- a/medmoe_amd/csrc/attention.hip
+++ b/medmoe_amd/csrc/attention.hip
@@ -8,20 +8,21 @@
 }
 
 template <int CNT, int RT>
-__device__ __forceinline__ void fill_rowmajor(char* lds, const bf16_t* src, long long row_stride, int n_valid, int tid) {
-  constexpr int PER = (CNT + RT - 1) / RT;
-  uint4 v[PER];
-#pragma unroll
-  for (int i = 0; i < PER; ++i) {
+__device__ __forceinline__ void fill_load(bf16x8_t (&v)[(CNT + RT - 1) / RT], const bf16_t* src, long long row_stride, int n_valid, int tid) {
+#pragma unroll
+  for (int i = 0; i < (CNT + RT - 1) / RT; ++i) {
     const int idx = min(tid + i * RT, CNT - 1);
     const int row = idx >> 3, c = idx & 7;
-    v[i] = *(const uint4*)(src + (long long)min(row, n_valid - 1) * row_stride + c * 8);
-  }
-#pragma unroll
-  for (int i = 0; i < PER; ++i) {
+    v[i] = *(const bf16x8_t*)(src + (long long)min(row, n_valid - 1) * row_stride + c * 8);
+  }
+}
+template <int CNT, int RT>
+__device__ __forceinline__ void fill_store(char* lds, const bf16x8_t (&v)[(CNT + RT - 1) / RT], int tid) {
+#pragma unroll
+  for (int i = 0; i < (CNT + RT - 1) / RT; ++i) {
     const int idx = tid + i * RT;
     const int row = idx >> 3, c = idx & 7;
-    if (idx < CNT) *(uint4*)(lds + row * 128 + ((c ^ (row & 7)) << 4)) = v[i];
+    if (idx < CNT) *(bf16x8_t*)(lds + row * 128 + ((c ^ (row & 7)) << 4)) = v[i];
   }
 }
 
@@ -75,6 +76,74 @@
   static constexpr int FILL = RMROWS * 8;
 };
 
+struct AttnItem {
+  int b, h, N;
+  long long row0;
+};
+__device__ __forceinline__ AttnItem attn_item(int item, int H, int Nmax, const int* __restrict__ seq_off) {
+  AttnItem it;
+  it.b = item / H;
+  it.h = item - it.b * H;
+  it.row0 = seq_off ? (long long)seq_off[it.b] : (long long)it.b * Nmax;
+  it.N = seq_off ? max(1, min(seq_off[it.b + 1] - seq_off[it.b], Nmax)) : Nmax;
+  return it;
+}
+template <int NKT, int NT, int NR>
+struct AttnStage {
+  using G = AttnGeom<NKT>;
+  static constexpr int PER = (G::FILL + NT - 1) / NT, RPT = (G::NKP + NT - 1) / NT;
+  bf16x8_t a[PER], b[PER];
+  float row[NR][RPT];
+  __device__ __forceinline__ void load(const bf16_t* s0, long long stride0, const bf16_t* s1, long long stride1,
+                                       const unsigned char* __restrict__ mask_row, const float* __restrict__ lse_row,
+                                       const float* __restrict__ delta_row, int N, int t) {
+    fill_load<G::FILL, NT>(a, s0, stride0, N, t);
+    fill_load<G::FILL, NT>(b, s1, stride1, N, t);
+    load_rows(mask_row, lse_row, delta_row, N, t);
+  }
+  __device__ __forceinline__ void load_rows(const unsigned char* __restrict__ mask_row, const float* __restrict__ lse_row,
+                                            const float* __restrict__ delta_row, int N, int t) {
+#pragma unroll
+    for (int j = 0; j < RPT; ++j) {
+      const int k = t + j * NT;
+      const bool valid = k < N;
+      row[0][j] = (valid && (!mask_row || mask_row[k])) ? 0.f : -INFINITY;
+      if constexpr (NR == 3) {
+        row[1][j] = valid ? lse_row[k] * 1.44269504088896f : INFINITY;
+        row[2][j] = valid ? delta_row[k] : 0.f;
+      }
+    }
+  }
+  __device__ __forceinline__ void store(char* img0, char* img1, float* rows, int t) const {
+    fill_store<G::FILL, NT>(img0, a, t);
+    fill_store<G::FILL, NT>(img1, b, t);
+    store_rows(rows, t);
+  }
+  __device__ __forceinline__ void store_rows(float* rows, int t) const {
+#pragma unroll
+    for (int j = 0; j < RPT; ++j) {
+      const int k = t + j * NT;
+#pragma unroll
+      for (int r = 0; r < NR; ++r)
+        if (k < G::NKP) rows[r * G::NKP + k] = row[r][j];
+    }
+  }
+};
+#define ATTN_HANDOVER(NR, s0, stride0, s1, stride1, mask_row, lse_row, delta_row, nN, img0, img1, rows)  \
+  {                                                                                                     \
+    int t = tid;                                                                                        \
+    asm volatile("" : "+v"(t));                                                                         \
+    AttnStage<NKT, RT, NR> st;                                                                          \
+    st.load_rows(mask_row, lse_row, delta_row, nN, t);                                                  \
+    fill_load<G::FILL, RT>(st.a, s0, stride0, nN, t);                                                   \
+    __syncthreads();                     \
+    fill_store<G::FILL, RT>(img0, st.a, t);                                                             \
+    st.store_rows(rows, t);                                                                             \
+    fill_load<G::FILL, RT>(st.a, s1, stride1, nN, t);                                                   \
+    fill_store<G::FILL, RT>(img1, st.a, t);                                                             \
+    __syncthreads();                                                                                    \
+  }
+
 #ifdef ATTN_TIMING
 __device__ unsigned long long g_attn_timing[8];
 #define ATTN_T(...) __VA_ARGS__
@@ -83,147 +152,169 @@
 #endif
 
 template <int NKT, bool MASKED, int RT>
-__global__ __launch_bounds__(RT, RT == 256 ? 2 : 4) void attn_fwd_kernel(const bf16_t* __restrict__ qkv, bf16_t* __restrict__ out,
+__global__ __launch_bounds__(RT, 4) void attn_fwd_kernel(const bf16_t* __restrict__ qkv, bf16_t* __restrict__ out,
                                                          float* __restrict__ lse, const unsigned char* __restrict__ key_mask,
-                                                         int Nmax, int H, float scale, const int* __restrict__ seq_off) {
+                                                         int Nmax, int H, float scale, const int* __restrict__ seq_off, int items) {
   using G = AttnGeom<NKT>;
+  static_assert(G::NKP <= RT, "one mask row element per thread");
   constexpr int CH = 8;
   constexpr int NCH = (NKT + CH - 1) / CH;
   __shared__ __attribute__((aligned(16))) char smem[2 * G::RM_BYTES + G::NKP * 4];
   char* sK = smem;
   char* sV = smem + G::RM_BYTES;
   float* sMask = (float*)(smem + 2 * G::RM_BYTES);
-  const int tid = threadIdx.x, lane = tid & 63, wid = tid >> 6;
-  const int b = blockIdx.x / H, h = blockIdx.x - b * H;
+  const int tid = threadIdx.x;
   const int D = H * HD;
   const long long rs = 3LL * D;
-  const long long row0 = seq_off ? (long long)seq_off[b] : (long long)b * Nmax;
-  const int N = seq_off ? max(1, min(seq_off[b + 1] - seq_off[b], Nmax)) : Nmax;
-  const bf16_t* base = qkv + row0 * rs + h * HD;
-
-  fill_rowmajor<G::FILL, RT>(sK, base + D, rs, N, tid);
-  fill_rowmajor<G::FILL, RT>(sV, base + 2 * D, rs, N, tid);
-  for (int k = tid; k < G::NKP; k += RT)
-    sMask[k] = (k < N && (!key_mask || key_mask[(long long)b * Nmax + k])) ? 0.f : -INFINITY;
-  __syncthreads();
-
-  const int fr = lane & 15, g = lane >> 4;
-  const int nqb = (N + 15) >> 4;
   const float c2 = scale * 1.44269504088896f;
+
+  int item = blockIdx.x;
+  AttnItem it = attn_item(item, H, Nmax, seq_off);
   bf16x8_t qf[2], qn[2];
   {
-    const int qc0 = min(wid * 16 + fr, N - 1);
+    const int lane = tid & 63, wid = tid >> 6, fr = lane & 15, g = lane >> 4;
+    const bf16_t* base = qkv + it.row0 * rs + it.h * HD;
+    AttnStage<NKT, RT, 1> st;
+    st.load(base + D, rs, base + 2 * D, rs, key_mask ? key_mask + (long long)it.b * Nmax : nullptr, nullptr, nullptr, it.N, tid);
+    const int qc0 = min(wid * 16 + fr, it.N - 1);
     qf[0] = load_frag_global(base, rs, qc0, g);
     qf[1] = load_frag_global(base, rs, qc0, 4 + g);
-  }
-  for (int qb = wid; qb < nqb; qb += RT / 64) {
-    const int q = qb * 16 + fr;
-    {
-      const int qcn = min((qb + RT / 64) * 16 + fr, N - 1);
-      qn[0] = load_frag_global(base, rs, qcn, g);
-      qn[1] = load_frag_global(base, rs, qcn, 4 + g);
-    }
-    float m = -INFINITY, lp = 0.f;
-    f32x4_t o[4];
-#pragma unroll
-    for (int nd = 0; nd < 4; ++nd) o[nd] = (f32x4_t){0.f, 0.f, 0.f, 0.f};
+    st.store(sK, sV, sMask, tid);
+  }
+  __syncthreads();
+  for (;;) {
+    int tl = tid;
+    asm volatile("" : "+v"(tl));
+    const int lane = tl & 63, wid = __builtin_amdgcn_readfirstlane(tl >> 6), fr = lane & 15, g = lane >> 4;
+    const int nitem = item + (int)gridDim.x;
+    const bool more = nitem < items;
+    AttnItem nx = it;
+    if (more) nx = attn_item(nitem, H, Nmax, seq_off);
+    const int b = it.b, h = it.h, N = it.N;
+    const long long row0 = it.row0;
+    const bf16_t* base = qkv + row0 * rs + h * HD;
+    const bf16_t* nbase = qkv + nx.row0 * rs + nx.h * HD;
+    const int nqb = (N + 15) >> 4;
+    if (more && wid >= nqb) {
+      const int qc0 = min(wid * 16 + fr, nx.N - 1);
+      qf[0] = load_frag_global(nbase, rs, qc0, g);
+      qf[1] = load_frag_global(nbase, rs, qc0, 4 + g);
+    }
+    for (int qb = wid; qb < nqb; qb += RT / 64) {
+      const int q = qb * 16 + fr;
+      {
+        const bool last = qb + RT / 64 >= nqb;
+        const int qcn = last ? min(wid * 16 + fr, nx.N - 1) : min((qb + RT / 64) * 16 + fr, N - 1);
+        const bf16_t* fb = last ? nbase : base;
+        qn[0] = load_frag_global(fb, rs, qcn, g);
+        qn[1] = load_frag_global(fb, rs, qcn, 4 + g);
+      }
+      float m = -INFINITY, lp = 0.f;
+      f32x4_t o[4];
+#pragma unroll
+      for (int nd = 0; nd < 4; ++nd) o[nd] = (f32x4_t){0.f, 0.f, 0.f, 0.f};
 #pragma unroll 1
-    for (int c = 0; c < NCH; ++c) {
-      const int kt0 = c * CH;
-      f32x4_t s[CH];
-#pragma unroll
-      for (int u = 0; u < CH; ++u) {
-        s[u] = (f32x4_t){0.f, 0.f, 0.f, 0.f};
-        if (kt0 + u < NKT) {
-          const char* kr = sK + ((kt0 + u) * 16 + fr) * 128;
-#pragma unroll
-          for (int ks = 0; ks < 2; ++ks) {
-            const bf16x8_t kf = *(const bf16x8_t*)(kr + (((ks * 4 + g) ^ (fr & 7)) << 4));
-            s[u] = __builtin_amdgcn_mfma_f32_16x16x32_bf16(kf, qf[ks], s[u], 0, 0, 0);
+      for (int c = 0; c < NCH; ++c) {
+        const int kt0 = c * CH;
+        f32x4_t s[CH];
+#pragma unroll
+        for (int u = 0; u < CH; ++u) {
+          s[u] = (f32x4_t){0.f, 0.f, 0.f, 0.f};
+          if (kt0 + u < NKT) {
+            const char* kr = sK + ((kt0 + u) * 16 + fr) * 128;
+#pragma unroll
+            for (int ks = 0; ks < 2; ++ks) {
+              const bf16x8_t kf = *(const bf16x8_t*)(kr + (((ks * 4 + g) ^ (fr & 7)) << 4));
+              s[u] = __builtin_amdgcn_mfma_f32_16x16x32_bf16(kf, qf[ks], s[u], 0, 0, 0);
+            }
           }
         }
-      }
-      float alpha;
-      f32x2_t l2 = {0.f, 0.f};
-      if constexpr (MASKED) {
-        float bm = -INFINITY;
-#pragma unroll
-        for (int u = 0; u < CH; ++u)
-          if (kt0 + u < NKT) {
-            const float4 mk = *(const float4*)(sMask + (kt0 + u) * 16 + g * 4);
-            const f32x2_t t0 = (f32x2_t){s[u][0], s[u][1]} * c2 + (f32x2_t){mk.x, mk.y};
-            const f32x2_t t1 = (f32x2_t){s[u][2], s[u][3]} * c2 + (f32x2_t){mk.z, mk.w};
-            s[u][0] = t0[0]; s[u][1] = t0[1]; s[u][2] = t1[0]; s[u][3] = t1[1];
-            bm = fmaxf(fmaxf(bm, fmaxf(t0[0], t0[1])), fmaxf(t1[0], t1[1]));
-          }
-        bm = fmaxf(bm, __shfl_xor(bm, 16, 64));
-        bm = fmaxf(bm, __shfl_xor(bm, 32, 64));
-        const float mn = fmaxf(m, bm);
-        const float ms = (mn == -INFINITY) ? 0.f : mn;
-        alpha = __builtin_amdgcn_exp2f(m - ms);
-        m = mn;
-#pragma unroll
-        for (int u = 0; u < CH; ++u)
-          if (kt0 + u < NKT) {
-            const f32x2_t d0 = (f32x2_t){s[u][0], s[u][1]} - ms, d1 = (f32x2_t){s[u][2], s[u][3]} - ms;
-            const f32x2_t e0 = {__builtin_amdgcn_exp2f(d0[0]), __builtin_amdgcn_exp2f(d0[1])};
-            const f32x2_t e1 = {__builtin_amdgcn_exp2f(d1[0]), __builtin_amdgcn_exp2f(d1[1])};
-            s[u][0] = e0[0]; s[u][1] = e0[1]; s[u][2] = e1[0]; s[u][3] = e1[1];
-            l2 += e0 + e1;
-          }
-      } else {
-        float bm = fmaxf(fmaxf(s[0][0], s[0][1]), fmaxf(s[0][2], s[0][3]));
-#pragma unroll
-        for (int u = 1; u < CH; ++u)
-          if (kt0 + u < NKT) bm = fmaxf(fmaxf(bm, fmaxf(s[u][0], s[u][1])), fmaxf(s[u][2], s[u][3]));
-        bm = fmaxf(bm, __shfl_xor(bm, 16, 64));
-        bm = fmaxf(bm, __shfl_xor(bm, 32, 64));
-        const float mn = fmaxf(m, bm * c2);
-        alpha = __builtin_amdgcn_exp2f(m - mn);
-        m = mn;
-        const float nm = -mn;
-#pragma unroll
-        for (int u = 0; u < CH; ++u)
-          if (kt0 + u < NKT) {
-            const f32x2_t d0 = (f32x2_t){s[u][0], s[u][1]} * c2 + nm, d1 = (f32x2_t){s[u][2], s[u][3]} * c2 + nm;
-            f32x2_t e0 = {__builtin_amdgcn_exp2f(d0[0]), __builtin_amdgcn_exp2f(d0[1])};
-            f32x2_t e1 = {__builtin_amdgcn_exp2f(d1[0]), __builtin_amdgcn_exp2f(d1[1])};
-            if ((kt0 + u) * 16 + 16 > N) {
-              const int k0 = (kt0 + u) * 16 + g * 4;
-              e0[0] = k0 < N ? e0[0] : 0.f; e0[1] = k0 + 1 < N ? e0[1] : 0.f;
-              e1[0] = k0 + 2 < N ? e1[0] : 0.f; e1[1] = k0 + 3 < N ? e1[1] : 0.f;
+        float alpha;
+        f32x2_t l2 = {0.f, 0.f};
+        if constexpr (MASKED) {
+          float bm = -INFINITY;
+#pragma unroll
+          for (int u = 0; u < CH; ++u)
+            if (kt0 + u < NKT) {
+              const float4 mk = *(const float4*)(sMask + (kt0 + u) * 16 + g * 4);
+              const f32x2_t t0 = (f32x2_t){s[u][0], s[u][1]} * c2 + (f32x2_t){mk.x, mk.y};
+              const f32x2_t t1 = (f32x2_t){s[u][2], s[u][3]} * c2 + (f32x2_t){mk.z, mk.w};
+              s[u][0] = t0[0]; s[u][1] = t0[1]; s[u][2] = t1[0]; s[u][3] = t1[1];
+              bm = fmaxf(fmaxf(bm, fmaxf(t0[0], t0[1])), fmaxf(t1[0], t1[1]));
             }
-            s[u][0] = e0[0]; s[u][1] = e0[1]; s[u][2] = e1[0]; s[u][3] = e1[1];
-            l2 += e0 + e1;
-          }
-      }
-      lp = lp * alpha + l2[0] + l2[1];
-#pragma unroll
-      for (int nd = 0; nd < 4; ++nd) {
-        if (c > 0) o[nd] *= alpha;
-#pragma unroll
-        for (int t = 0; t < CH / 2; ++t)
-          if (kt0 + 2 * t < NKT) {
-            const bf16x8_t pf = pack_frag(s[2 * t], s[2 * t + 1]);
-            const bf16x8_t vf = tr_frag(sV, (kt0 + 2 * t) * 16, nd * 16, lane);
-            o[nd] = __builtin_amdgcn_mfma_f32_16x16x32_bf16(vf, pf, o[nd], 0, 0, 0);
-          }
-      }
-    }
-    float l = lp;
-    l += __shfl_xor(l, 16, 64);
-    l += __shfl_xor(l, 32, 64);
-    const float inv = l > 0.f ? 1.f / l : 0.f;
-    if (q < N) {
-      if (g == 0) lse[((long long)b * H + h) * Nmax + q] = (m + __log2f(l)) * 0.693147180559945f;
-#pragma unroll
-      for (int nd = 0; nd < 4; ++nd) {
-        const f32x4_t v = o[nd] * inv;
-        uint2 pk; pk.x = pack2bf(v[0], v[1]); pk.y = pack2bf(v[2], v[3]);
-        *(uint2*)(out + (row0 + q) * D + h * HD + nd * 16 + g * 4) = pk;
-      }
-    }
-    qf[0] = qn[0]; qf[1] = qn[1];
+          bm = fmaxf(bm, __shfl_xor(bm, 16, 64));
+          bm = fmaxf(bm, __shfl_xor(bm, 32, 64));
+          const float mn = fmaxf(m, bm);
+          const float ms = (mn == -INFINITY) ? 0.f : mn;
+          alpha = __builtin_amdgcn_exp2f(m - ms);
+          m = mn;
+#pragma unroll
+          for (int u = 0; u < CH; ++u)
+            if (kt0 + u < NKT) {
+              const f32x2_t d0 = (f32x2_t){s[u][0], s[u][1]} - ms, d1 = (f32x2_t){s[u][2], s[u][3]} - ms;
+              const f32x2_t e0 = {__builtin_amdgcn_exp2f(d0[0]), __builtin_amdgcn_exp2f(d0[1])};
+              const f32x2_t e1 = {__builtin_amdgcn_exp2f(d1[0]), __builtin_amdgcn_exp2f(d1[1])};
+              s[u][0] = e0[0]; s[u][1] = e0[1]; s[u][2] = e1[0]; s[u][3] = e1[1];
+              l2 += e0 + e1;
+            }
+        } else {
+          float bm = fmaxf(fmaxf(s[0][0], s[0][1]), fmaxf(s[0][2], s[0][3]));
+#pragma unroll
+          for (int u = 1; u < CH; ++u)
+            if (kt0 + u < NKT) bm = fmaxf(fmaxf(bm, fmaxf(s[u][0], s[u][1])), fmaxf(s[u][2], s[u][3]));
+          bm = fmaxf(bm, __shfl_xor(bm, 16, 64));
+          bm = fmaxf(bm, __shfl_xor(bm, 32, 64));
+          const float mn = fmaxf(m, bm * c2);
+          alpha = __builtin_amdgcn_exp2f(m - mn);
+          m = mn;
+          const float nm = -mn;
+#pragma unroll
+          for (int u = 0; u < CH; ++u)
+            if (kt0 + u < NKT) {
+              const f32x2_t d0 = (f32x2_t){s[u][0], s[u][1]} * c2 + nm, d1 = (f32x2_t){s[u][2], s[u][3]} * c2 + nm;
+              f32x2_t e0 = {__builtin_amdgcn_exp2f(d0[0]), __builtin_amdgcn_exp2f(d0[1])};
+              f32x2_t e1 = {__builtin_amdgcn_exp2f(d1[0]), __builtin_amdgcn_exp2f(d1[1])};
+              if ((kt0 + u) * 16 + 16 > N) {
+                const int k0 = (kt0 + u) * 16 + g * 4;
+                e0[0] = k0 < N ? e0[0] : 0.f; e0[1] = k0 + 1 < N ? e0[1] : 0.f;
+                e1[0] = k0 + 2 < N ? e1[0] : 0.f; e1[1] = k0 + 3 < N ? e1[1] : 0.f;
+              }
+              s[u][0] = e0[0]; s[u][1] = e0[1]; s[u][2] = e1[0]; s[u][3] = e1[1];
+              l2 += e0 + e1;
+            }
+        }
+        lp = lp * alpha + l2[0] + l2[1];
+#pragma unroll
+        for (int nd = 0; nd < 4; ++nd) {
+          if (c > 0) o[nd] *= alpha;
+#pragma unroll
+          for (int t = 0; t < CH / 2; ++t)
+            if (kt0 + 2 * t < NKT) {
+              const bf16x8_t pf = pack_frag(s[2 * t], s[2 * t + 1]);
+              const bf16x8_t vf = tr_frag(sV, (kt0 + 2 * t) * 16, nd * 16, lane);
+              o[nd] = __builtin_amdgcn_mfma_f32_16x16x32_bf16(vf, pf, o[nd], 0, 0, 0);
+            }
+        }
+      }
+      float l = lp;
+      l += __shfl_xor(l, 16, 64);
+      l += __shfl_xor(l, 32, 64);
+      const float inv = l > 0.f ? 1.f / l : 0.f;
+      if (q < N) {
+        if (g == 0) lse[((long long)b * H + h) * Nmax + q] = (m + __log2f(l)) * 0.693147180559945f;
+#pragma unroll
+        for (int nd = 0; nd < 4; ++nd) {
+          const f32x4_t v = o[nd] * inv;
+          uint2 pk; pk.x = pack2bf(v[0], v[1]); pk.y = pack2bf(v[2], v[3]);
+          *(uint2*)(out + (row0 + q) * D + h * HD + nd * 16 + g * 4) = pk;
+        }
+      }
+      qf[0] = qn[0]; qf[1] = qn[1];
+    }
+    if (!more) break;
+    ATTN_HANDOVER(1, nbase + D, rs, nbase + 2 * D, rs, key_mask ? key_mask + (long long)nx.b * Nmax : nullptr, nullptr, nullptr, nx.N, sK, sV, sMask)
+    it = nx;
+    item = nitem;
   }
 }
 
@@ -232,114 +323,146 @@
                                                           const bf16_t* __restrict__ dout, const float* __restrict__ lse,
                                                           const unsigned char* __restrict__ key_mask,
                                                           bf16_t* __restrict__ dqkv, float* __restrict__ delta,
-                                                          int Nmax, int H, float scale, const int* __restrict__ seq_off) {
+                                                          int Nmax, int H, float scale, const int* __restrict__ seq_off, int items) {
   using G = AttnGeom<NKT>;
+  static_assert(G::NKP <= RT, "one mask row element per thread");
   __shared__ __attribute__((aligned(16))) char smem[2 * G::RM_BYTES + G::NKP * 4];
   char* sK = smem;
   char* sV = smem + G::RM_BYTES;
   float* sMask = (float*)(smem + 2 * G::RM_BYTES);
-  const int tid = threadIdx.x, lane = tid & 63, wid = tid >> 6;
-  const int b = blockIdx.x / H, h = blockIdx.x - b * H;
+  const int tid = threadIdx.x;
   const int D = H * HD;
   const long long rs = 3LL * D;
-  const long long row0 = seq_off ? (long long)seq_off[b] : (long long)b * Nmax;
-  const int N = seq_off ? max(1, min(seq_off[b + 1] - seq_off[b], Nmax)) : Nmax;
-  const bf16_t* base = qkv + row0 * rs + h * HD;
-  const bf16_t* obase = o + row0 * D + h * HD;
-  const bf16_t* dobase = dout + row0 * D + h * HD;
-
-  fill_rowmajor<G::FILL, RT>(sK, base + D, rs, N, tid);
-  fill_rowmajor<G::FILL, RT>(sV, base + 2 * D, rs, N, tid);
-  for (int k = tid; k < G::NKP; k += RT)
-    sMask[k] = (k < N && (!key_mask || key_mask[(long long)b * Nmax + k])) ? 0.f : -INFINITY;
-  __syncthreads();
-
-  const int fr = lane & 15, g = lane >> 4;
-  const int nqb = (N + 15) >> 4;
+  const float c2 = scale * 1.44269504088896f;
+
   bf16x8_t qf[2], dof[2], of[2], qn[2], don[2], on[2];
+  float lq, lqn;
+  int item = blockIdx.x;
+  AttnItem it = attn_item(item, H, Nmax, seq_off);
   {
-    const int qc0 = min(wid * 16 + fr, N - 1);
+    const int lane = tid & 63, wid = tid >> 6, fr = lane & 15, g = lane >> 4;
+    const bf16_t* base = qkv + it.row0 * rs + it.h * HD;
+    AttnStage<NKT, RT, 1> st;
+    st.load(base + D, rs, base + 2 * D, rs, key_mask ? key_mask + (long long)it.b * Nmax : nullptr, nullptr, nullptr, it.N, tid);
+    st.store(sK, sV, sMask, tid);
+    const int qc0 = min(wid * 16 + fr, it.N - 1);
+    const long long ro = it.row0 * D + it.h * HD;
 #pragma unroll
     for (int ks = 0; ks < 2; ++ks) {
       qf[ks] = load_frag_global(base, rs, qc0, ks * 4 + g);
-      dof[ks] = load_frag_global(dobase, D, qc0, ks * 4 + g);
-      of[ks] = load_frag_global(obase, D, qc0, ks * 4 + g);
-    }
-  }
-  for (int qb = wid; qb < nqb; qb += RT / 64) {
-    const int q = qb * 16 + fr;
-    const int qc = min(q, N - 1);
-    {
-      const int qcn = min((qb + RT / 64) * 16 + fr, N - 1);
+      dof[ks] = load_frag_global(dout + ro, D, qc0, ks * 4 + g);
+      of[ks] = load_frag_global(o + ro, D, qc0, ks * 4 + g);
+    }
+    lq = lse[((long long)it.b * H + it.h) * Nmax + qc0];
+  }
+  __syncthreads();
+  for (;;) {
+    int tl = tid;
+    asm volatile("" : "+v"(tl));
+    const int lane = tl & 63, wid = __builtin_amdgcn_readfirstlane(tl >> 6), fr = lane & 15, g = lane >> 4;
+    const int nitem = item + (int)gridDim.x;
+    const bool more = nitem < items;
+    AttnItem nx = it;
+    if (more) nx = attn_item(nitem, H, Nmax, seq_off);
+    const int b = it.b, h = it.h, N = it.N;
+    const long long row0 = it.row0;
+    const bf16_t* base = qkv + row0 * rs + h * HD;
+    const bf16_t* nbase = qkv + nx.row0 * rs + nx.h * HD;
+    const long long ro = row0 * D + h * HD, nro = nx.row0 * D + nx.h * HD;
+    const long long lrow = ((long long)b * H + h) * Nmax, nlrow = ((long long)nx.b * H + nx.h) * Nmax;
+    const int nqb = (N + 15) >> 4;
+    if (more && wid >= nqb) {
+      const int qc0 = min(wid * 16 + fr, nx.N - 1);
 #pragma unroll
       for (int ks = 0; ks < 2; ++ks) {
-        qn[ks] = load_frag_global(base, rs, qcn, ks * 4 + g);
-        don[ks] = load_frag_global(dobase, D, qcn, ks * 4 + g);
-        on[ks] = load_frag_global(obase, D, qcn, ks * 4 + g);
-      }
-    }
-    float dl = 0.f;
-#pragma unroll
-    for (int ks = 0; ks < 2; ++ks)
-#pragma unroll
-      for (int e = 0; e < 8; ++e) dl += (float)dof[ks][e] * (float)of[ks][e];
-    dl += __shfl_xor(dl, 16, 64);
-    dl += __shfl_xor(dl, 32, 64);
-    const float c2 = scale * 1.44269504088896f;
-    const float nL2 = -lse[((long long)b * H + h) * Nmax + qc] * 1.44269504088896f;
-    if (g == 0 && q < N) delta[((long long)b * H + h) * Nmax + q] = dl;
-
-    f32x4_t acc[4];
-#pragma unroll
-    for (int nd = 0; nd < 4; ++nd) acc[nd] = (f32x4_t){0.f, 0.f, 0.f, 0.f};
+        qf[ks] = load_frag_global(nbase, rs, qc0, ks * 4 + g);
+        dof[ks] = load_frag_global(dout + nro, D, qc0, ks * 4 + g);
+        of[ks] = load_frag_global(o + nro, D, qc0, ks * 4 + g);
+      }
+      lq = lse[nlrow + qc0];
+    }
+    for (int qb = wid; qb < nqb; qb += RT / 64) {
+      const int q = qb * 16 + fr;
+      {
+        const bool last = qb + RT / 64 >= nqb;
+        const int qcn = last ? min(wid * 16 + fr, nx.N - 1) : min((qb + RT / 64) * 16 + fr, N - 1);
+        const bf16_t* fb = last ? nbase : base;
+        const long long fo = last ? nro : ro;
+#pragma unroll
+        for (int ks = 0; ks < 2; ++ks) {
+          qn[ks] = load_frag_global(fb, rs, qcn, ks * 4 + g);
+          don[ks] = load_frag_global(dout + fo, D, qcn, ks * 4 + g);
+          on[ks] = load_frag_global(o + fo, D, qcn, ks * 4 + g);
+        }
+        lqn = lse[(last ? nlrow : lrow) + qcn];
+      }
+      float dl = 0.f;
+#pragma unroll
+      for (int ks = 0; ks < 2; ++ks)
+#pragma unroll
+        for (int e = 0; e < 8; ++e) dl += (float)dof[ks][e] * (float)of[ks][e];
+      dl += __shfl_xor(dl, 16, 64);
+      dl += __shfl_xor(dl, 32, 64);
+      const float nL2 = -lq * 1.44269504088896f;
+      if (g == 0 && q < N) delta[lrow + q] = dl;
+
+      f32x4_t acc[4];
+#pragma unroll
+      for (int nd = 0; nd < 4; ++nd) acc[nd] = (f32x4_t){0.f, 0.f, 0.f, 0.f};
 #pragma unroll 1
-    for (int t = 0; t < G::KS; ++t) {
-      f32x4_t ds[2];
-#pragma unroll
-      for (int u = 0; u < 2; ++u) {
-        const int kt = 2 * t + u;
-        ds[u] = (f32x4_t){0.f, 0.f, 0.f, 0.f};
-        if (kt < NKT) {
-          f32x4_t s = {0.f, 0.f, 0.f, 0.f}, dp = {0.f, 0.f, 0.f, 0.f};
-          const char* kr = sK + (kt * 16 + fr) * 128;
-          const char* vr = sV + (kt * 16 + fr) * 128;
-#pragma unroll
-          for (int ks = 0; ks < 2; ++ks) {
-            const int off = ((ks * 4 + g) ^ (fr & 7)) << 4;
-            s = __builtin_amdgcn_mfma_f32_16x16x32_bf16(*(const bf16x8_t*)(kr + off), qf[ks], s, 0, 0, 0);
-            dp = __builtin_amdgcn_mfma_f32_16x16x32_bf16(*(const bf16x8_t*)(vr + off), dof[ks], dp, 0, 0, 0);
+      for (int t = 0; t < G::KS; ++t) {
+        f32x4_t ds[2];
+#pragma unroll
+        for (int u = 0; u < 2; ++u) {
+          const int kt = 2 * t + u;
+          ds[u] = (f32x4_t){0.f, 0.f, 0.f, 0.f};
+          if (kt < NKT) {
+            f32x4_t s = {0.f, 0.f, 0.f, 0.f}, dp = {0.f, 0.f, 0.f, 0.f};
+            const char* kr = sK + (kt * 16 + fr) * 128;
+            const char* vr = sV + (kt * 16 + fr) * 128;
+#pragma unroll
+            for (int ks = 0; ks < 2; ++ks) {
+              const int off = ((ks * 4 + g) ^ (fr & 7)) << 4;
+              s = __builtin_amdgcn_mfma_f32_16x16x32_bf16(*(const bf16x8_t*)(kr + off), qf[ks], s, 0, 0, 0);
+              dp = __builtin_amdgcn_mfma_f32_16x16x32_bf16(*(const bf16x8_t*)(vr + off), dof[ks], dp, 0, 0, 0);
+            }
+            if (MASKED || kt * 16 + 16 > N) {
+              const float4 mk = *(const float4*)(sMask + kt * 16 + g * 4);
+              const float mkv[4] = {mk.x, mk.y, mk.z, mk.w};
+#pragma unroll
+              for (int r = 0; r < 4; ++r) ds[u][r] = __builtin_amdgcn_exp2f(s[r] * c2 + (mkv[r] + nL2)) * (dp[r] - dl);
+            } else {
+              const f32x2_t t0 = (f32x2_t){s[0], s[1]} * c2 + nL2, t1 = (f32x2_t){s[2], s[3]} * c2 + nL2;
+              const f32x2_t g0 = (f32x2_t){dp[0], dp[1]} - dl, g1 = (f32x2_t){dp[2], dp[3]} - dl;
+              const f32x2_t d0 = (f32x2_t){__builtin_amdgcn_exp2f(t0[0]), __builtin_amdgcn_exp2f(t0[1])} * g0;
+              const f32x2_t d1 = (f32x2_t){__builtin_amdgcn_exp2f(t1[0]), __builtin_amdgcn_exp2f(t1[1])} * g1;
+              ds[u] = (f32x4_t){d0[0], d0[1], d1[0], d1[1]};
+            }
           }
-          if (MASKED || kt * 16 + 16 > N) {
-            const float4 mk = *(const float4*)(sMask + kt * 16 + g * 4);
-            const float mkv[4] = {mk.x, mk.y, mk.z, mk.w};
-#pragma unroll
-            for (int r = 0; r < 4; ++r) ds[u][r] = __builtin_amdgcn_exp2f(s[r] * c2 + (mkv[r] + nL2)) * (dp[r] - dl);
-          } else {
-            const f32x2_t t0 = (f32x2_t){s[0], s[1]} * c2 + nL2, t1 = (f32x2_t){s[2], s[3]} * c2 + nL2;
-            const f32x2_t g0 = (f32x2_t){dp[0], dp[1]} - dl, g1 = (f32x2_t){dp[2], dp[3]} - dl;
-            const f32x2_t d0 = (f32x2_t){__builtin_amdgcn_exp2f(t0[0]), __builtin_amdgcn_exp2f(t0[1])} * g0;
-            const f32x2_t d1 = (f32x2_t){__builtin_amdgcn_exp2f(t1[0]), __builtin_amdgcn_exp2f(t1[1])} * g1;
-            ds[u] = (f32x4_t){d0[0], d0[1], d1[0], d1[1]};
-          }
-        }
-      }
-      const bf16x8_t dsf = pack_frag(ds[0], ds[1]);
-#pragma unroll
-      for (int nd = 0; nd < 4; ++nd) {
-        const bf16x8_t ktf = tr_frag(sK, t * 32, nd * 16, lane);
-        acc[nd] = __builtin_amdgcn_mfma_f32_16x16x32_bf16(ktf, dsf, acc[nd], 0, 0, 0);
-      }
-    }
-    if (q < N) {
-#pragma unroll
-      for (int nd = 0; nd < 4; ++nd) {
-        const f32x4_t v = acc[nd] * scale;
-        uint2 pk; pk.x = pack2bf(v[0], v[1]); pk.y = pack2bf(v[2], v[3]);
-        *(uint2*)(dqkv + (row0 + q) * rs + h * HD + nd * 16 + g * 4) = pk;
-      }
-    }
-#pragma unroll
-    for (int ks = 0; ks < 2; ++ks) { qf[ks] = qn[ks]; dof[ks] = don[ks]; of[ks] = on[ks]; }
+        }
+        const bf16x8_t dsf = pack_frag(ds[0], ds[1]);
+#pragma unroll
+        for (int nd = 0; nd < 4; ++nd) {
+          const bf16x8_t ktf = tr_frag(sK, t * 32, nd * 16, lane);
+          acc[nd] = __builtin_amdgcn_mfma_f32_16x16x32_bf16(ktf, dsf, acc[nd], 0, 0, 0);
+        }
+      }
+      if (q < N) {
+#pragma unroll
+        for (int nd = 0; nd < 4; ++nd) {
+          const f32x4_t v = acc[nd] * scale;
+          uint2 pk; pk.x = pack2bf(v[0], v[1]); pk.y = pack2bf(v[2], v[3]);
+          *(uint2*)(dqkv + (row0 + q) * rs + h * HD + nd * 16 + g * 4) = pk;
+        }
+      }
+#pragma unroll
+      for (int ks = 0; ks < 2; ++ks) { qf[ks] = qn[ks]; dof[ks] = don[ks]; of[ks] = on[ks]; }
+      lq = lqn;
+    }
+    if (!more) break;
+    ATTN_HANDOVER(1, nbase + D, rs, nbase + 2 * D, rs, key_mask ? key_mask + (long long)nx.b * Nmax : nullptr, nullptr, nullptr, nx.N, sK, sV, sMask)
+    it = nx;
+    item = nitem;
   }
 }
 
@@ -348,117 +471,144 @@
                                                            const float* __restrict__ lse, const float* __restrict__ delta,
                                                            const unsigned char* __restrict__ key_mask,
                                                            bf16_t* __restrict__ dqkv, int Nmax, int H, float scale,
-                                                           const int* __restrict__ seq_off) {
+                                                           const int* __restrict__ seq_off, int items) {
   using G = AttnGeom<NKT>;
+  static_assert(G::NKP <= RT, "one element of the mask / lse / delta rows per thread");
   __shared__ __attribute__((aligned(16))) char smem[2 * G::RM_BYTES + G::NKP * 12];
   char* sQ = smem;
   char* sDO = smem + G::RM_BYTES;
   float* sMask = (float*)(smem + 2 * G::RM_BYTES);
   float* sLse = sMask + G::NKP;
   float* sDelta = sLse + G::NKP;
-  const int tid = threadIdx.x, lane = tid & 63, wid = tid >> 6;
-  const int b = blockIdx.x / H, h = blockIdx.x - b * H;
+  const int tid = threadIdx.x;
   const int D = H * HD;
   const long long rs = 3LL * D;
-  const long long row0 = seq_off ? (long long)seq_off[b] : (long long)b * Nmax;
-  const int N = seq_off ? max(1, min(seq_off[b + 1] - seq_off[b], Nmax)) : Nmax;
-  const bf16_t* base = qkv + row0 * rs + h * HD;
-  const bf16_t* dobase = dout + row0 * D + h * HD;
-
-  fill_rowmajor<G::FILL, RT>(sQ, base, rs, N, tid);
-  fill_rowmajor<G::FILL, RT>(sDO, dobase, D, N, tid);
-  for (int k = tid; k < G::NKP; k += RT) {
-    const bool valid = k < N;
-    sMask[k] = (valid && (!key_mask || key_mask[(long long)b * Nmax + k])) ? 0.f : -INFINITY;
-    sLse[k] = valid ? lse[((long long)b * H + h) * Nmax + k] * 1.44269504088896f : INFINITY;
-    sDelta[k] = valid ? delta[((long long)b * H + h) * Nmax + k] : 0.f;
-  }
-  __syncthreads();
-
-  const int fr = lane & 15, g = lane >> 4;
-  const int nkb = (N + 15) >> 4;
+  const float c2 = scale * 1.44269504088896f;
+
   bf16x8_t kf[2], vf[2], kn[2], vn[2];
+  int item = blockIdx.x;
+  AttnItem it = attn_item(item, H, Nmax, seq_off);
   {
-    const int kc0 = min(wid * 16 + fr, N - 1);
+    const int lane = tid & 63, wid = tid >> 6, fr = lane & 15, g = lane >> 4;
+    const bf16_t* base = qkv + it.row0 * rs + it.h * HD;
+    const long long lrow = ((long long)it.b * H + it.h) * Nmax;
+    AttnStage<NKT, RT, 3> st;
+    st.load(base, rs, dout + it.row0 * D + it.h * HD, D, key_mask ? key_mask + (long long)it.b * Nmax : nullptr, lse + lrow, delta + lrow, it.N, tid);
+    st.store(sQ, sDO, sMask, tid);
+    const int kc0 = min(wid * 16 + fr, it.N - 1);
 #pragma unroll
     for (int ks = 0; ks < 2; ++ks) {
       kf[ks] = load_frag_global(base + D, rs, kc0, ks * 4 + g);
       vf[ks] = load_frag_global(base + 2 * D, rs, kc0, ks * 4 + g);
     }
   }
-  for (int kb = wid; kb < nkb; kb += RT / 64) {
-    const int key = kb * 16 + fr;
+  __syncthreads();
+  for (;;) {
+    int tl = tid;
+    asm volatile("" : "+v"(tl));
+    const int lane = tl & 63, wid = __builtin_amdgcn_readfirstlane(tl >> 6), fr = lane & 15, g = lane >> 4;
+    const int nitem = item + (int)gridDim.x;
+    const bool more = nitem < items;
+    AttnItem nx = it;
+    if (more) nx = attn_item(nitem, H, Nmax, seq_off);
+    const int h = it.h, N = it.N;
+    const long long row0 = it.row0;
+    const bf16_t* base = qkv + row0 * rs + h * HD;
+    const bf16_t* nbase = qkv + nx.row0 * rs + nx.h * HD;
+    const int nkb = (N + 15) >> 4;
+    if (more && wid >= nkb) {
+      const int kc0 = min(wid * 16 + fr, nx.N - 1);
+#pragma unroll
+      for (int ks = 0; ks < 2; ++ks) {
+        kf[ks] = load_frag_global(nbase + D, rs, kc0, ks * 4 + g);
+        vf[ks] = load_frag_global(nbase + 2 * D, rs, kc0, ks * 4 + g);
+      }
+    }
+    for (int kb = wid; kb < nkb; kb += RT / 64) {
+      const int key = kb * 16 + fr;
+      {
+        const bool last = kb + RT / 64 >= nkb;
+        const int kcn = last ? min(wid * 16 + fr, nx.N - 1) : min((kb + RT / 64) * 16 + fr, N - 1);
+        const bf16_t* fb = last ? nbase : base;
+#pragma unroll
+        for (int ks = 0; ks < 2; ++ks) {
+          kn[ks] = load_frag_global(fb + D, rs, kcn, ks * 4 + g);
+          vn[ks] = load_frag_global(fb + 2 * D, rs, kcn, ks * 4 + g);
+        }
+      }
+      const float mk = sMask[kb * 16 + fr];
+      f32x4_t dk[4], dv[4];
+#pragma unroll
+      for (int nd = 0; nd < 4; ++nd) { dk[nd] = (f32x4_t){0.f, 0.f, 0.f, 0.f}; dv[nd] = (f32x4_t){0.f, 0.f, 0.f, 0.f}; }
+
+#pragma unroll 1
+      for (int t = 0; t < G::KS; ++t) {
+        f32x4_t pp[2], dss[2];
+#pragma unroll
+        for (int u = 0; u < 2; ++u) {
+          const int qt = 2 * t + u;
+          if (qt < NKT) {
+            f32x4_t s = {0.f, 0.f, 0.f, 0.f}, dp = {0.f, 0.f, 0.f, 0.f};
+            const char* qr = sQ + (qt * 16 + fr) * 128;
+            const char* dr = sDO + (qt * 16 + fr) * 128;
+#pragma unroll
+            for (int ks = 0; ks < 2; ++ks) {
+              const int off = ((ks * 4 + g) ^ (fr & 7)) << 4;
+              s = __builtin_amdgcn_mfma_f32_16x16x32_bf16(*(const bf16x8_t*)(qr + off), kf[ks], s, 0, 0, 0);
+              dp = __builtin_amdgcn_mfma_f32_16x16x32_bf16(*(const bf16x8_t*)(dr + off), vf[ks], dp, 0, 0, 0);
+            }
+            const float4 L4 = *(const float4*)(sLse + qt * 16 + g * 4);
+            const float4 D4 = *(const float4*)(sDelta + qt * 16 + g * 4);
+            const float Lv[4] = {L4.x, L4.y, L4.z, L4.w}, Dv[4] = {D4.x, D4.y, D4.z, D4.w};
+            const f32x2_t t0 = (f32x2_t){s[0], s[1]} * c2 + (mk - (f32x2_t){Lv[0], Lv[1]});
+            const f32x2_t t1 = (f32x2_t){s[2], s[3]} * c2 + (mk - (f32x2_t){Lv[2], Lv[3]});
+            const f32x2_t p0 = {__builtin_amdgcn_exp2f(t0[0]), __builtin_amdgcn_exp2f(t0[1])};
+            const f32x2_t p1 = {__builtin_amdgcn_exp2f(t1[0]), __builtin_amdgcn_exp2f(t1[1])};
+            const f32x2_t d0 = p0 * ((f32x2_t){dp[0], dp[1]} - (f32x2_t){Dv[0], Dv[1]});
+            const f32x2_t d1 = p1 * ((f32x2_t){dp[2], dp[3]} - (f32x2_t){Dv[2], Dv[3]});
+            pp[u] = (f32x4_t){p0[0], p0[1], p1[0], p1[1]};
+            dss[u] = (f32x4_t){d0[0], d0[1], d1[0], d1[1]};
+          } else {
+            pp[u] = (f32x4_t){0.f, 0.f, 0.f, 0.f};
+            dss[u] = (f32x4_t){0.f, 0.f, 0.f, 0.f};
+          }
+        }
+        const bf16x8_t pf = pack_frag(pp[0], pp[1]);
+        const bf16x8_t dsf = pack_frag(dss[0], dss[1]);
+#pragma unroll
+        for (int nd = 0; nd < 4; ++nd) {
+          const bf16x8_t dot = tr_frag(sDO, t * 32, nd * 16, lane);
+          const bf16x8_t qt_ = tr_frag(sQ, t * 32, nd * 16, lane);
+          dv[nd] = __builtin_amdgcn_mfma_f32_16x16x32_bf16(dot, pf, dv[nd], 0, 0, 0);
+          dk[nd] = __builtin_amdgcn_mfma_f32_16x16x32_bf16(qt_, dsf, dk[nd], 0, 0, 0);
+        }
+      }
+      if (key < N) {
+        bf16_t* row = dqkv + (row0 + key) * rs + h * HD;
+#pragma unroll
+        for (int nd = 0; nd < 4; ++nd) {
+          const f32x4_t kv = dk[nd] * scale;
+          uint2 pk; pk.x = pack2bf(kv[0], kv[1]); pk.y = pack2bf(kv[2], kv[3]);
+          *(uint2*)(row + D + nd * 16 + g * 4) = pk;
+          pk.x = pack2bf(dv[nd][0], dv[nd][1]); pk.y = pack2bf(dv[nd][2], dv[nd][3]);
+          *(uint2*)(row + 2 * D + nd * 16 + g * 4) = pk;
+        }
+      }
+#pragma unroll
+      for (int ks = 0; ks < 2; ++ks) { kf[ks] = kn[ks]; vf[ks] = vn[ks]; }
+    }
+    if (!more) break;
     {
-      const int kcn = min((kb + RT / 64) * 16 + fr, N - 1);
-#pragma unroll
-      for (int ks = 0; ks < 2; ++ks) {
-        kn[ks] = load_frag_global(base + D, rs, kcn, ks * 4 + g);
-        vn[ks] = load_frag_global(base + 2 * D, rs, kcn, ks * 4 + g);
-      }
-    }
-    const float mk = sMask[kb * 16 + fr];
-    const float c2 = scale * 1.44269504088896f;
-    f32x4_t dk[4], dv[4];
-#pragma unroll
-    for (int nd = 0; nd < 4; ++nd) { dk[nd] = (f32x4_t){0.f, 0.f, 0.f, 0.f}; dv[nd] = (f32x4_t){0.f, 0.f, 0.f, 0.f}; }
-
-#pragma unroll 1
-    for (int t = 0; t < G::KS; ++t) {
-      f32x4_t pp[2], dss[2];
-#pragma unroll
-      for (int u = 0; u < 2; ++u) {
-        const int qt = 2 * t + u;
-        if (qt < NKT) {
-          f32x4_t s = {0.f, 0.f, 0.f, 0.f}, dp = {0.f, 0.f, 0.f, 0.f};
-          const char* qr = sQ + (qt * 16 + fr) * 128;
-          const char* dr = sDO + (qt * 16 + fr) * 128;
-#pragma unroll
-          for (int ks = 0; ks < 2; ++ks) {
-            const int off = ((ks * 4 + g) ^ (fr & 7)) << 4;
-            s = __builtin_amdgcn_mfma_f32_16x16x32_bf16(*(const bf16x8_t*)(qr + off), kf[ks], s, 0, 0, 0);
-            dp = __builtin_amdgcn_mfma_f32_16x16x32_bf16(*(const bf16x8_t*)(dr + off), vf[ks], dp, 0, 0, 0);
-          }
-          const float4 L4 = *(const float4*)(sLse + qt * 16 + g * 4);
-          const float4 D4 = *(const float4*)(sDelta + qt * 16 + g * 4);
-          const float Lv[4] = {L4.x, L4.y, L4.z, L4.w}, Dv[4] = {D4.x, D4.y, D4.z, D4.w};
-          const f32x2_t t0 = (f32x2_t){s[0], s[1]} * c2 + (mk - (f32x2_t){Lv[0], Lv[1]});
-          const f32x2_t t1 = (f32x2_t){s[2], s[3]} * c2 + (mk - (f32x2_t){Lv[2], Lv[3]});
-          const f32x2_t p0 = {__builtin_amdgcn_exp2f(t0[0]), __builtin_amdgcn_exp2f(t0[1])};
-          const f32x2_t p1 = {__builtin_amdgcn_exp2f(t1[0]), __builtin_amdgcn_exp2f(t1[1])};
-          const f32x2_t d0 = p0 * ((f32x2_t){dp[0], dp[1]} - (f32x2_t){Dv[0], Dv[1]});
-          const f32x2_t d1 = p1 * ((f32x2_t){dp[2], dp[3]} - (f32x2_t){Dv[2], Dv[3]});
-          pp[u] = (f32x4_t){p0[0], p0[1], p1[0], p1[1]};
-          dss[u] = (f32x4_t){d0[0], d0[1], d1[0], d1[1]};
-        } else {
-          pp[u] = (f32x4_t){0.f, 0.f, 0.f, 0.f};
-          dss[u] = (f32x4_t){0.f, 0.f, 0.f, 0.f};
-        }
-      }
-      const bf16x8_t pf = pack_frag(pp[0], pp[1]);
-      const bf16x8_t dsf = pack_frag(dss[0], dss[1]);
-#pragma unroll
-      for (int nd = 0; nd < 4; ++nd) {
-        const bf16x8_t dot = tr_frag(sDO, t * 32, nd * 16, lane);
-        const bf16x8_t qt_ = tr_frag(sQ, t * 32, nd * 16, lane);
-        dv[nd] = __builtin_amdgcn_mfma_f32_16x16x32_bf16(dot, pf, dv[nd], 0, 0, 0);
-        dk[nd] = __builtin_amdgcn_mfma_f32_16x16x32_bf16(qt_, dsf, dk[nd], 0, 0, 0);
-      }
-    }
-    if (key < N) {
-      bf16_t* row = dqkv + (row0 + key) * rs + h * HD;
-#pragma unroll
-      for (int nd = 0; nd < 4; ++nd) {
-        const f32x4_t kv = dk[nd] * scale;
-        uint2 pk; pk.x = pack2bf(kv[0], kv[1]); pk.y = pack2bf(kv[2], kv[3]);
-        *(uint2*)(row + D + nd * 16 + g * 4) = pk;
-        pk.x = pack2bf(dv[nd][0], dv[nd][1]); pk.y = pack2bf(dv[nd][2], dv[nd][3]);
-        *(uint2*)(row + 2 * D + nd * 16 + g * 4) = pk;
-      }
-    }
-#pragma unroll
-    for (int ks = 0; ks < 2; ++ks) { kf[ks] = kn[ks]; vf[ks] = vn[ks]; }
-  }
-}
+      const long long nlrow = ((long long)nx.b * H + nx.h) * Nmax;
+      ATTN_HANDOVER(3, nbase, rs, dout + nx.row0 * D + nx.h * HD, D, key_mask ? key_mask + (long long)nx.b * Nmax : nullptr, lse + nlrow, delta + nlrow, nx.N,
+                    sQ, sDO, sMask)
+    }
+    it = nx;
+    item = nitem;
+  }
+}
+
+#undef ATTN_HANDOVER
 
 #define SB 64
 #define SB_BYTES (SB * 128)
@@ -850,6 +1000,35 @@
 int g_attn_resident = 1;
 int g_attn_rt13 = 0;
 
+int g_attn_grid_cap = 0;
+static int g_attn_last_grid[3] = {0, 0, 0};
+extern "C" int medmoe_attn_last_grid(int which) { return which >= 0 && which < 3 ? g_attn_last_grid[which] : MM_ERR_ARG; }
+
+static int attn_cu_count() {
+  static int cus = 0;
+  if (!cus) {
+    int dev = 0, n = 0;
+    if (hipGetDevice(&dev) != hipSuccess || hipDeviceGetAttribute(&n, hipDeviceAttributeMultiprocessorCount, dev) != hipSuccess || n < 1) n = 1;
+    cus = n;
+  }
+  return cus;
+}
+template <typename KernelT>
+static int attn_grid(KernelT kernel, int threads, int items, int which, int& slot, bool persist) {
+  if (!slot) {
+    int n = 0;
+    if (hipOccupancyMaxActiveBlocksPerMultiprocessor(&n, kernel, threads, 0) != hipSuccess || n < 1) n = 1;
+    slot = n;
+  }
+  const long long full = (long long)attn_cu_count() * slot;
+  const long long cap = g_attn_grid_cap > 0 ? g_attn_grid_cap : persist ? full : items;
+  const int grid = (int)(cap < items ? cap : items);
+  g_attn_last_grid[which] = grid;
+  return grid;
+}
+
+static bool attn_persist_auto(int nkt, bool forward, int items) { return items >= 4096 && (forward ? nkt == 5 : (nkt == 5 || nkt == 13)); }
+
 static int pick_nkt(int N) {
   if (N <= 80) return 5;
   if (N <= 208) return 13;
@@ -858,20 +1037,35 @@
   return 0;
 }
 
+template <int K, bool MASKED, int RT>
+static void launch_fwd_m(const void* qkv, void* out, float* lse, const unsigned char* key_mask, const int* seq_off, int B, int N, int H, float scale,
+                         hipStream_t stream) {
+  static int slot = 0;
+  const int grid = attn_grid(attn_fwd_kernel<K, MASKED, RT>, RT, B * H, 0, slot, attn_persist_auto(K, true, B * H));
+  hipLaunchKernelGGL((attn_fwd_kernel<K, MASKED, RT>), dim3(grid), dim3(RT), 0, stream, (const bf16_t*)qkv, (bf16_t*)out, lse, key_mask, N, H, scale,
+                     seq_off, B * H);
+}
 template <int K, int RT>
 static void launch_fwd(const void* qkv, void* out, float* lse, const unsigned char* key_mask, int B, int N, int H, float scale, hipStream_t stream) {
-  if (key_mask) hipLaunchKernelGGL((attn_fwd_kernel<K, true, RT>), dim3(B * H), dim3(RT), 0, stream, (const bf16_t*)qkv, (bf16_t*)out, lse, key_mask, N, H, scale, (const int*)nullptr);
-  else hipLaunchKernelGGL((attn_fwd_kernel<K, false, RT>), dim3(B * H), dim3(RT), 0, stream, (const bf16_t*)qkv, (bf16_t*)out, lse, key_mask, N, H, scale, (const int*)nullptr);
+  if (key_mask) launch_fwd_m<K, true, RT>(qkv, out, lse, key_mask, nullptr, B, N, H, scale, stream);
+  else launch_fwd_m<K, false, RT>(qkv, out, lse, key_mask, nullptr, B, N, H, scale, stream);
+}
+template <int K, bool MASKED, int RT>
+static void launch_bwd_m(const void* qkv, const void* out, const void* dout, const float* lse, const unsigned char* key_mask, const int* seq_off,
+                         void* dqkv, float* delta, int B, int N, int H, float scale, hipStream_t stream) {
+  static int slot_dq = 0, slot_dkv = 0;
+  const int gq = attn_grid(attn_bwd_dq_kernel<K, MASKED, RT>, RT, B * H, 1, slot_dq, attn_persist_auto(K, false, B * H));
+  hipLaunchKernelGGL((attn_bwd_dq_kernel<K, MASKED, RT>), dim3(gq), dim3(RT), 0, stream, (const bf16_t*)qkv, (const bf16_t*)out,
+                     (const bf16_t*)dout, lse, key_mask, (bf16_t*)dqkv, delta, N, H, scale, seq_off, B * H);
+  const int gk = attn_grid(attn_bwd_dkv_kernel<K, RT>, RT, B * H, 2, slot_dkv, attn_persist_auto(K, false, B * H));
+  hipLaunchKernelGGL((attn_bwd_dkv_kernel<K, RT>), dim3(gk), dim3(RT), 0, stream, (const bf16_t*)qkv, (const bf16_t*)dout, lse, delta,
+                     key_mask, (bf16_t*)dqkv, N, H, scale, seq_off, B * H);
 }
 template <int K, int RT>
 static void launch_bwd(const void* qkv, const void* out, const void* dout, const float* lse, const unsigned char* key_mask, void* dqkv,
                        float* delta, int B, int N, int H, float scale, hipStream_t stream) {
-  if (key_mask) hipLaunchKernelGGL((attn_bwd_dq_kernel<K, true, RT>), dim3(B * H), dim3(RT), 0, stream, (const bf16_t*)qkv, (const bf16_t*)out,
-                                   (const bf16_t*)dout, lse, key_mask, (bf16_t*)dqkv, delta, N, H, scale, (const int*)nullptr);
-  else hipLaunchKernelGGL((attn_bwd_dq_kernel<K, false, RT>), dim3(B * H), dim3(RT), 0, stream, (const bf16_t*)qkv, (const bf16_t*)out,
-                          (const bf16_t*)dout, lse, key_mask, (bf16_t*)dqkv, delta, N, H, scale, (const int*)nullptr);
-  hipLaunchKernelGGL((attn_bwd_dkv_kernel<K, RT>), dim3(B * H), dim3(RT), 0, stream, (const bf16_t*)qkv, (const bf16_t*)dout, lse, delta,
-                     key_mask, (bf16_t*)dqkv, N, H, scale, (const int*)nullptr);
+  if (key_mask) launch_bwd_m<K, true, RT>(qkv, out, dout, lse, key_mask, nullptr, dqkv, delta, B, N, H, scale, stream);
+  else launch_bwd_m<K, false, RT>(qkv, out, dout, lse, key_mask, nullptr, dqkv, delta, B, N, H, scale, stream);
 }
 
 extern "C" int medmoe_attn_fwd(const void* qkv, void* out, float* lse, const unsigned char* key_mask,
@@ -900,8 +1094,7 @@
                                       hipStream_t stream) {
   if (!qkv || !out || !lse || !seq_off) return MM_ERR_ARG;
   if (head_dim != HD || B <= 0 || H <= 0 || Nmax <= 0 || Nmax > 80) return MM_ERR_SHAPE;
-  hipLaunchKernelGGL((attn_fwd_kernel<5, false, 256>), dim3(B * H), dim3(256), 0, stream, (const bf16_t*)qkv, (bf16_t*)out, lse,
-                     (const unsigned char*)nullptr, Nmax, H, 0.125f, seq_off);
+  launch_fwd_m<5, false, 256>(qkv, out, lse, nullptr, seq_off, B, Nmax, H, 0.125f, stream);
   return mm_check_launch();
 }
 
@@ -934,9 +1127,6 @@
                                       float* delta, int B, int Nmax, int H, int head_dim, hipStream_t stream) {
   if (!qkv || !out || !dout || !lse || !seq_off || !dqkv || !delta) return MM_ERR_ARG;
   if (head_dim != HD || B <= 0 || H <= 0 || Nmax <= 0 || Nmax > 80) return MM_ERR_SHAPE;
-  hipLaunchKernelGGL((attn_bwd_dq_kernel<5, false, 256>), dim3(B * H), dim3(256), 0, stream, (const bf16_t*)qkv, (const bf16_t*)out,
-                     (const bf16_t*)dout, lse, (const unsigned char*)nullptr, (bf16_t*)dqkv, delta, Nmax, H, 0.125f, seq_off);
-  hipLaunchKernelGGL((attn_bwd_dkv_kernel<5, 256>), dim3(B * H), dim3(256), 0, stream, (const bf16_t*)qkv, (const bf16_t*)dout, lse, delta,
-                     (const unsigned char*)nullptr, (bf16_t*)dqkv, Nmax, H, 0.125f, seq_off);
+  launch_bwd_m<5, false, 256>(qkv, out, dout, lse, nullptr, seq_off, dqkv, delta, B, Nmax, H, 0.125f, stream);
   return mm_check_launch();
 }
diff --git a/medmoe_amd/csrc/gemm.hip b/medmoe_amd/csrc/gemm.hip
--- a/medmoe_amd/csrc/gemm.hip
+++ b/medmoe_amd/csrc/gemm.hip
@@ -38,6 +38,7 @@
 extern int g_attn_resident;
 extern int g_sa_rows;
 extern int g_attn_rt13;
+extern int g_attn_grid_cap;
 static int g_last_nt_kernel = -1;
 extern "C" int medmoe_last_gemm_nt_kernel() { return g_last_nt_kernel; }
 extern int g_ln_one_row;
@@ -56,6 +57,7 @@
   if (key == 9 && value >= 64) { g_tn_min_rows = value; return MM_OK; }
   if (key == 12) { g_scores_skip_epi = value; return MM_OK; }
   if (key == 15 && (value == 0 || value == 448 || value == 512)) { g_attn_rt13 = value; return MM_OK; }
+  if (key == 18 && value >= 0) { g_attn_grid_cap = value; return MM_OK; }
   if (key == 13 && value >= 0) { g_sa_rows = value; return MM_OK; }
   if (key == 11) { g_attn_resident = value; return MM_OK; }
   if (key == 10 && value >= 0) { g_tn_rows4w = value; return MM_OK; }
```

Result: no change. 4832 pairs/s, median of 6 (+0.5%).
